# HKUST-Aerial-Robotics/VINS-Mobile

Hardware: AMD Instinct MI355X
Metric: VIO frames/sec (KLT+window solve), 640x480/150 feats/W=10 (higher is better)
Workload: dtype f64 (solve) / u8+i32+f32 (KLT)

## Files before the change

vins-mobile_amd/csrc/vio_frontend.hip:

```cpp
#include <hip/hip_runtime.h>

#include <type_traits>

#include <math.h>
#include <stdint.h>
#include <stdio.h>
#include <string.h>

#include <algorithm>
#include <condition_variable>
#include <memory>
#include <mutex>
#include <thread>
#include <vector>

#include "vio_amd.h"
#include "vio_device.h"
#include "vio_pool.h"

namespace {

constexpr int kMaxLevels = 4;
constexpr int kMaxCap = 512;
constexpr int kWin = 21;
constexpr int kWBits = 14;
constexpr int kMaxRadius = 128;

struct LevelDims {
  int rows[kMaxLevels], cols[kMaxLevels];
  size_t off[kMaxLevels];
  size_t pyr_bytes;
  int levels;
};

__device__ __forceinline__ int reflect101(int p, int len) {
  p = p < 0 ? -p : p;
  p = p >= len ? 2 * len - 2 - p : p;
  return p;
}
__device__ __forceinline__ int descale(int x, int n) { return (x + (1 << (n - 1))) >> n; }

constexpr int kPdW = 64, kPdH = 8;
__global__ __launch_bounds__(256) void pyr_down_kernel(const uint8_t *src_base, uint8_t *dst_base, size_t seq_stride,
                                                       int srows, int scols, int drows, int dcols) {
  constexpr int SW = 2 * kPdW + 4, SH = 2 * kPdH + 4;
  __shared__ int patch[SH][SW + 1];
  __shared__ int hsum[SH][kPdW + 1];
  const uint8_t *src = src_base + (size_t)blockIdx.z * seq_stride;
  uint8_t *dst = dst_base + (size_t)blockIdx.z * seq_stride;
  const int ox = blockIdx.x * kPdW, oy = blockIdx.y * kPdH;
  const int tid = threadIdx.x;
  for (int e = tid; e < SH * SW; e += 256) {
    int ly = e / SW, lx = e - ly * SW;
    int y = reflect101(min(2 * oy + ly - 2, 2 * srows - 2), srows), x = reflect101(min(2 * ox + lx - 2, 2 * scols - 2), scols);
    patch[ly][lx] = src[(size_t)y * scols + x];
  }
  __syncthreads();
  for (int e = tid; e < SH * kPdW; e += 256) {
    int ly = e / kPdW, lx = e - ly * kPdW;
    const int *r = &patch[ly][2 * lx];
    hsum[ly][lx] = r[0] + 4 * r[1] + 6 * r[2] + 4 * r[3] + r[4];
  }
  __syncthreads();
  for (int e = tid; e < kPdH * kPdW; e += 256) {
    int ly = e / kPdW, lx = e - ly * kPdW;
    int x = ox + lx, y = oy + ly;
    if (x < dcols && y < drows) {
      int v = hsum[2 * ly][lx] + 4 * hsum[2 * ly + 1][lx] + 6 * hsum[2 * ly + 2][lx] + 4 * hsum[2 * ly + 3][lx] + hsum[2 * ly + 4][lx];
      dst[(size_t)y * dcols + x] = (uint8_t)((v + 128) >> 8);
    }
  }
}

inline float lk_eps_screen(double eps_sq) { return nextafterf((float)(eps_sq * (1.0 + 1e-5)), INFINITY); }
struct LkParams {
  LevelDims ld;
  int cap;
  int max_count;
  float epsilon_sq_f;
  double epsilon_sq;
  float min_eig;
  const uint8_t *prev0, *next0;
  size_t stride0;
};

__device__ __forceinline__ int wave_sum_i32(int v) {
  v += __builtin_amdgcn_update_dpp(0, v, 0x111, 0xf, 0xf, false);
  v += __builtin_amdgcn_update_dpp(0, v, 0x112, 0xf, 0xf, false);
  v += __builtin_amdgcn_update_dpp(0, v, 0x114, 0xf, 0xf, false);
  v += __builtin_amdgcn_update_dpp(0, v, 0x118, 0xf, 0xf, false);
  v += __builtin_amdgcn_update_dpp(0, v, 0x142, 0xa, 0xf, false);
  v += __builtin_amdgcn_update_dpp(0, v, 0x143, 0xc, 0xf, false);
  return __builtin_amdgcn_readlane(v, 63);
}
__device__ __forceinline__ double wave_sum_exact(int p) {
  int lo = p & 0xffff, hi = p >> 16;
  int slo = wave_sum_i32(lo), shi = wave_sum_i32(hi);
  return (double)shi * 65536.0 + (double)slo;
}

__device__ __forceinline__ void lk_weights(float a, float b, int &iw00, int &iw01, int &iw10, int &iw11) {
  iw00 = __float2int_rn((1.f - a) * (1.f - b) * (1 << kWBits));
  iw01 = __float2int_rn(a * (1.f - b) * (1 << kWBits));
  iw10 = __float2int_rn((1.f - a) * b * (1 << kWBits));
  iw11 = (1 << kWBits) - iw00 - iw01 - iw10;
}

constexpr int kIP = kWin + 3;
constexpr int kDP = kWin + 1;
constexpr int kJMargin = 3;
constexpr int kJP = kWin + 1 + 2 * kJMargin;
constexpr int kJS = 43;
constexpr int kIS = kIP + 1;
struct LkWaveLds {
  union {
    struct {
      uint32_t I[kIP][kIS];
      short2 dI[kDP][kDP];
    };
    uint32_t J[kJP][kJS];
  };
};
typedef short lk_s2 __attribute__((ext_vector_type(2)));
typedef unsigned short lk_us2 __attribute__((ext_vector_type(2)));

struct __attribute__((packed)) LkU32 {
  uint32_t v;
};
__device__ __forceinline__ uint32_t lk_load4(const uint8_t *p) { return reinterpret_cast<const LkU32 *>(p)->v; }
__device__ __forceinline__ void lk_pairs(uint32_t cur, uint32_t next, uint32_t w[4]) {
  w[0] = __builtin_amdgcn_perm(0u, cur, 0x0c010c00u);
  w[1] = __builtin_amdgcn_perm(0u, cur, 0x0c020c01u);
  w[2] = __builtin_amdgcn_perm(0u, cur, 0x0c030c02u);
  w[3] = __builtin_amdgcn_perm(next, cur, 0x0c040c03u);
}

__device__ __forceinline__ void wave_lds_fence() {
  __builtin_amdgcn_fence(__ATOMIC_RELEASE, "wavefront");
  __builtin_amdgcn_wave_barrier();
  __builtin_amdgcn_fence(__ATOMIC_ACQUIRE, "wavefront");
}

__device__ __forceinline__ bool wave_all_small(int p, int q, int r = 0) {
  const bool small = (unsigned)(p + (1 << 24)) < (1u << 25) && (unsigned)(q + (1 << 24)) < (1u << 25) && (unsigned)(r + (1 << 24)) < (1u << 25);
  return __builtin_amdgcn_ballot_w64(!small) == 0ull;
}
__device__ __forceinline__ void wave_sum_exact2(int p, int q, float &sp, float &sq) {
  if (wave_all_small(p, q)) {
    int u[2] = {p, q};
#define VIO_DPPS(ctrl, rmask)                                                  \
  {                                                                            \
    const int t0 = __builtin_amdgcn_update_dpp(0, u[0], ctrl, rmask, 0xf, false); \
    const int t1 = __builtin_amdgcn_update_dpp(0, u[1], ctrl, rmask, 0xf, false); \
    u[0] += t0, u[1] += t1;                                                    \
  }
    VIO_DPPS(0x111, 0xf) VIO_DPPS(0x112, 0xf) VIO_DPPS(0x114, 0xf) VIO_DPPS(0x118, 0xf) VIO_DPPS(0x142, 0xa) VIO_DPPS(0x143, 0xc)
#undef VIO_DPPS
    sp = (float)__builtin_amdgcn_readlane(u[0], 63), sq = (float)__builtin_amdgcn_readlane(u[1], 63);
    return;
  }
  int a = p & 0xffff, b = q & 0xffff, c = p >> 16, d = q >> 16;
#define VIO_DPP4(ctrl, rmask)                                              \
  {                                                                        \
    const int ta = __builtin_amdgcn_update_dpp(0, a, ctrl, rmask, 0xf, false); \
    const int tb = __builtin_amdgcn_update_dpp(0, b, ctrl, rmask, 0xf, false); \
    const int tc = __builtin_amdgcn_update_dpp(0, c, ctrl, rmask, 0xf, false); \
    const int td = __builtin_amdgcn_update_dpp(0, d, ctrl, rmask, 0xf, false); \
    a += ta, b += tb, c += tc, d += td;                                    \
  }
  VIO_DPP4(0x111, 0xf) VIO_DPP4(0x112, 0xf) VIO_DPP4(0x114, 0xf) VIO_DPP4(0x118, 0xf) VIO_DPP4(0x142, 0xa) VIO_DPP4(0x143, 0xc)
#undef VIO_DPP4
  const int sa = __builtin_amdgcn_readlane(a, 63), sb = __builtin_amdgcn_readlane(b, 63), sc = __builtin_amdgcn_readlane(c, 63),
            sd = __builtin_amdgcn_readlane(d, 63);
  sp = (float)sc * 65536.f + (float)sa, sq = (float)sd * 65536.f + (float)sb;
}

__device__ __forceinline__ void wave_sum_exact3(int p, int q, int r, float &sp, float &sq, float &sr) {
  if (wave_all_small(p, q, r)) {
    int w[3] = {p, q, r};
#define VIO_DPPS3(ctrl, rmask)                                                                                       \
  {                                                                                                                   \
    int t[3];                                                                                                         \
    _Pragma("unroll") for (int k = 0; k < 3; k++) t[k] = __builtin_amdgcn_update_dpp(0, w[k], ctrl, rmask, 0xf, false); \
    _Pragma("unroll") for (int k = 0; k < 3; k++) w[k] += t[k];                                                       \
  }
    VIO_DPPS3(0x111, 0xf) VIO_DPPS3(0x112, 0xf) VIO_DPPS3(0x114, 0xf) VIO_DPPS3(0x118, 0xf) VIO_DPPS3(0x142, 0xa) VIO_DPPS3(0x143, 0xc)
#undef VIO_DPPS3
    sp = (float)__builtin_amdgcn_readlane(w[0], 63), sq = (float)__builtin_amdgcn_readlane(w[1], 63), sr = (float)__builtin_amdgcn_readlane(w[2], 63);
    return;
  }
  int u[3] = {p, q, r};
#define VIO_DPPN(N, arr, ctrl, rmask)                                               \
  {                                                                                 \
    int t[N];                                                                       \
    _Pragma("unroll") for (int k = 0; k < N; k++) t[k] = __builtin_amdgcn_update_dpp(0, arr[k], ctrl, rmask, 0xf, false); \
    _Pragma("unroll") for (int k = 0; k < N; k++) arr[k] += t[k];                   \
  }
  VIO_DPPN(3, u, 0x111, 0xf) VIO_DPPN(3, u, 0x112, 0xf) VIO_DPPN(3, u, 0x114, 0xf) VIO_DPPN(3, u, 0x118, 0xf)
  int v[6] = {u[0] & 0xffff, u[1] & 0xffff, u[2] & 0xffff, u[0] >> 16, u[1] >> 16, u[2] >> 16};
  VIO_DPPN(6, v, 0x142, 0xa) VIO_DPPN(6, v, 0x143, 0xc)
#undef VIO_DPPN
  int s[6];
#pragma unroll
  for (int k = 0; k < 6; k++) s[k] = __builtin_amdgcn_readlane(v[k], 63);
  sp = (float)s[3] * 65536.f + (float)s[0], sq = (float)s[4] * 65536.f + (float)s[1], sr = (float)s[5] * 65536.f + (float)s[2];
}

template <bool STATS = false>
__global__ __launch_bounds__(256, 6) void lk_track_kernel(const uint8_t *prev_pyr, const uint8_t *next_pyr, LkParams P,
                                                       const int *n_pts, const float *prev_pts, float *next_pts,
                                                       uint8_t *status, float *err, unsigned long long *stats) {
  __shared__ LkWaveLds lds_all[4];
  const int seq = blockIdx.y;
  const int wave = threadIdx.x >> 6, lane = threadIdx.x & 63;
  const int pt = blockIdx.x * (blockDim.x >> 6) + wave;
  if (pt >= n_pts[seq]) return;
  LkWaveLds &L = lds_all[wave];
  const uint8_t *pp = prev_pyr + (size_t)seq * P.ld.pyr_bytes, *np = next_pyr + (size_t)seq * P.ld.pyr_bytes;
  const size_t pidx = ((size_t)seq * P.cap + pt) * 2;
  const float ptx = prev_pts[pidx], pty = prev_pts[pidx + 1];
  const float half = (kWin - 1) * 0.5f;
  const float FLT_SCALE = 1.f / (1 << 20);
  constexpr int NPX = (kWin * kWin + 63) / 64;
  const int wy0 = min(lane / kWin, 2), wx0 = lane % kWin;
  const int joff = wy0 * kJS + wx0;
  bool st = true;
  float er = 0.f;
  float nxx = 0.f, nxy = 0.f;
  const int max_level = P.ld.levels - 1;
  for (int level = max_level; level >= 0; level--) {
    const int rows = P.ld.rows[level], cols = P.ld.cols[level];
    const uint8_t *I = pp + P.ld.off[level], *J = np + P.ld.off[level];
    if (level == 0) {
      if (P.prev0) I = P.prev0 + (size_t)seq * P.stride0;
      if (P.next0) J = P.next0 + (size_t)seq * P.stride0;
    }
    const float scale = __int_as_float((127 - level) << 23);
    float px = ptx * scale, py = pty * scale;
    float qx, qy;
    if (level == max_level) qx = px, qy = py;
    else qx = nxx * 2.f, qy = nxy * 2.f;
    nxx = qx, nxy = qy;
    px -= half, py -= half;
    int ipx = (int)floorf(px), ipy = (int)floorf(py);
    if (ipx < -kWin || ipx >= cols || ipy < -kWin || ipy >= rows) {
      if (level == 0) st = false, er = 0.f;
      continue;
    }
    float a = px - ipx, b = py - ipy;
    int iw00, iw01, iw10, iw11;
    lk_weights(a, b, iw00, iw01, iw10, iw11);
    wave_lds_fence();
    if (ipx >= 1 && ipx + kIP - 1 <= cols && ipy >= 1 && ipy + kIP - 1 <= rows) {
      const int r = lane / 6, d = lane - 6 * r;
      constexpr int TI = (kIP + 9) / 10;
      uint32_t curs[TI];
#pragma unroll
      for (int t = 0; t < TI; t++) {
        const int ly = r + 10 * t;
        curs[t] = lk_load4(I + (unsigned)(__mul24(ipy - 1 + (ly < kIP ? ly : 0), cols) + ipx - 1 + 4 * d));
      }
#pragma unroll
      for (int t = 0; t < TI; t++) {
        const int ly = r + 10 * t;
        const bool ok = lane < 60 && ly < kIP;
        const uint32_t cur = curs[t];
        uint32_t next = (uint32_t)__builtin_amdgcn_update_dpp(0, (int)cur, 0x130, 0xf, 0xf, false);
        if (d == 5) next = cur >> 24;
        uint32_t w4[4];
        lk_pairs(cur, next, w4);
        if (ok) {
#pragma unroll
          for (int k = 0; k < 4; k++) L.I[ly][4 * d + k] = w4[k];
        }
      }
    } else {
      const int lx = lane & 31;
      const int x = reflect101(ipx - 1 + min(lx, kIP - 1), cols);
      constexpr int RPT = 2, TB = kIP / RPT;
      static_assert(kIP % RPT == 0, "whole trips");
      int vs[TB];
#pragma unroll
      for (int t = 0; t < TB; t++) {
        const int s_y0 = __builtin_amdgcn_readfirstlane(ipy) - 1 + RPT * t;
        const int ro_a = reflect101(s_y0, rows) * cols, ro_b = reflect101(s_y0 + 1, rows) * cols;
        vs[t] = I[(unsigned)(((lane >> 5) ? ro_b : ro_a) + x)];
      }
#pragma unroll
      for (int t = 0; t < TB; t++) {
        const int ly = (lane >> 5) + RPT * t, v = vs[t];
        const int vr = __builtin_amdgcn_update_dpp(0, v, 0x130, 0xf, 0xf, false);
        if (lx < kIP) L.I[ly][lx] = (uint32_t)v | ((uint32_t)vr << 16);
      }
    }
    wave_lds_fence();
    constexpr int SEG = 5, NSEG = 5, NCP = kDP / 2;
    static_assert(kDP % 2 == 0 && NCP * NSEG <= 64 && SEG * NSEG >= kDP && kDP >= SEG, "column pairs x segments");
    const bool inside = ipx >= 0 && ipx + kDP <= cols && ipy >= 0 && ipy + kDP <= rows;
    if (lane < NCP * NSEG) {
      const int seg = lane / NCP, cp = lane - NCP * seg, c = 2 * cp;
      const int r0 = seg * SEG < kDP - SEG ? seg * SEG : kDP - SEG;
      const uint32_t *Ip = &L.I[0][0] + (__mul24(r0, kIS) + c);
      uint32_t *Dp = reinterpret_cast<uint32_t *>(&L.dI[0][0]) + (__mul24(r0, kDP) + c);
      const lk_s2 k3 = {3, 3}, k10 = {10, 10};
      auto walk = [&](auto checked) {
        const unsigned ok0 = (unsigned)(ipx + c) < (unsigned)cols, ok1 = (unsigned)(ipx + c + 1) < (unsigned)cols;
        lk_s2 P0[SEG + 2], P1[SEG + 2], P2[SEG + 2];
#pragma unroll
        for (int r = 0; r < SEG + 2; r++)
          __builtin_memcpy(&P0[r], Ip + r * kIS, 4), __builtin_memcpy(&P1[r], Ip + r * kIS + 1, 4), __builtin_memcpy(&P2[r], Ip + r * kIS + 2, 4);
        lk_s2 h[SEG + 2], v[SEG + 2];
#pragma unroll
        for (int r = 0; r < SEG + 2; r++) h[r] = P2[r] - P0[r], v[r] = (P0[r] + P2[r]) * k3 + P1[r] * k10;
#pragma unroll
        for (int r = 2; r < SEG + 2; r++) {
          const lk_s2 dx = (h[r - 2] + h[r]) * k3 + h[r - 1] * k10, dy = v[r] - v[r - 2];
          uint32_t ux, uy;
          __builtin_memcpy(&ux, &dx, 4), __builtin_memcpy(&uy, &dy, 4);
          uint32_t d0 = __builtin_amdgcn_perm(uy, ux, 0x05040100u), d1 = __builtin_amdgcn_perm(uy, ux, 0x07060302u);
          if (decltype(checked)::value) {
            const unsigned rok = (unsigned)(ipy + r0 + r - 2) < (unsigned)rows;
            d0 &= 0u - (ok0 & rok), d1 &= 0u - (ok1 & rok);
          }
          Dp[(r - 2) * kDP] = d0, Dp[(r - 2) * kDP + 1] = d1;
        }
      };
      if (inside) walk(std::false_type{});
      else walk(std::true_type{});
    }
    wave_lds_fence();
    constexpr int NPP = (NPX + 1) / 2;
    const lk_s2 sw_top = {(short)iw00, (short)iw01}, sw_bot = {(short)iw10, (short)iw11};
    lk_s2 IxP[NPP], IyP[NPP];
    int Ic[NPX];
    int p11 = 0, p12 = 0, p22 = 0;
#pragma unroll
    for (int h = 0; h < NPP; h++) IxP[h] = IyP[h] = lk_s2{0, 0};
#pragma unroll
    for (int q = 0; q < NPX; q++) {
      const int y = wy0 + 3 * q, x = wx0;
      lk_s2 it, ib;
      __builtin_memcpy(&it, &L.I[y + 1][x + 1], 4);
      __builtin_memcpy(&ib, &L.I[y + 2][x + 1], 4);
      const int ival = __builtin_amdgcn_sdot2(it, sw_top, __builtin_amdgcn_sdot2(ib, sw_bot, 1 << (kWBits - 5 - 1), false), false) >> (kWBits - 5);
      uint32_t d00, d01, d10, d11;
      __builtin_memcpy(&d00, &L.dI[y][x], 4), __builtin_memcpy(&d01, &L.dI[y][x + 1], 4);
      __builtin_memcpy(&d10, &L.dI[y + 1][x], 4), __builtin_memcpy(&d11, &L.dI[y + 1][x + 1], 4);
      const uint32_t xt = __builtin_amdgcn_perm(d01, d00, 0x05040100u), yt = __builtin_amdgcn_perm(d01, d00, 0x07060302u);
      const uint32_t xb = __builtin_amdgcn_perm(d11, d10, 0x05040100u), yb = __builtin_amdgcn_perm(d11, d10, 0x07060302u);
      lk_s2 sxt, syt, sxb, syb;
      __builtin_memcpy(&sxt, &xt, 4), __builtin_memcpy(&syt, &yt, 4), __builtin_memcpy(&sxb, &xb, 4), __builtin_memcpy(&syb, &yb, 4);
      int ixval = __builtin_amdgcn_sdot2(sxt, sw_top, __builtin_amdgcn_sdot2(sxb, sw_bot, 1 << (kWBits - 1), false), false) >> kWBits;
      int iyval = __builtin_amdgcn_sdot2(syt, sw_top, __builtin_amdgcn_sdot2(syb, sw_bot, 1 << (kWBits - 1), false), false) >> kWBits;
      if (lane >= 3 * kWin) ixval = iyval = 0;
      Ic[q] = (1 << (kWBits - 5 - 1)) - (int)((unsigned)ival << (kWBits - 5));
      if (q & 1) IxP[q >> 1].y = (short)ixval, IyP[q >> 1].y = (short)iyval;
      else IxP[q >> 1].x = (short)ixval, IyP[q >> 1].x = (short)iyval;
      p11 += ixval * ixval, p12 += ixval * iyval, p22 += iyval * iyval;
    }
    float f11, f12, f22;
    wave_sum_exact3(p11, p12, p22, f11, f12, f22);
    float A11 = f11 * FLT_SCALE, A12 = f12 * FLT_SCALE, A22 = f22 * FLT_SCALE;
    float D = A11 * A22 - A12 * A12;
    float minEig = (A22 + A11 - sqrtf((A11 - A22) * (A11 - A22) + 4.f * A12 * A12)) / (2 * kWin * kWin);
    if (minEig < P.min_eig || D < 1.1920929e-07f) {
      if (level == 0) st = false;
      continue;
    }
    D = 1.f / D;
    qx -= half, qy -= half;
    float pdx = 0.f, pdy = 0.f;
    int jox = 0, joy = 0;
    bool j_staged = false;
    auto stage_j = [&](int iqx, int iqy) {
      jox = iqx - kJMargin, joy = iqy - kJMargin;
      wave_lds_fence();
      if (jox >= 0 && jox + kJP <= cols && joy >= 0 && joy + kJP <= rows) {
        const int r = lane / 7, d = lane - 7 * r;
        constexpr int TJ = (kJP + 8) / 9;
        uint32_t curs[TJ];
#pragma unroll
        for (int t = 0; t < TJ; t++) {
          const int ly = r + 9 * t;
          curs[t] = lk_load4(J + (unsigned)(__mul24(joy + (ly < kJP ? ly : 0), cols) + jox + 4 * d));
        }
#pragma unroll
        for (int t = 0; t < TJ; t++) {
          const int ly = r + 9 * t;
          const bool ok = lane < 63 && ly < kJP;
          const uint32_t cur = curs[t];
          uint32_t next = (uint32_t)__builtin_amdgcn_update_dpp(0, (int)cur, 0x130, 0xf, 0xf, false);
          if (d == 6) next = cur >> 24;
          uint32_t w4[4];
          lk_pairs(cur, next, w4);
          if (ok) {
#pragma unroll
            for (int k = 0; k < 4; k++) L.J[ly][4 * d + k] = w4[k];
          }
        }
      } else {
        const int lx = lane & 31;
        const int x = reflect101(min(max(jox + min(lx, kJP - 1), -cols + 1), 2 * cols - 2), cols);
        constexpr int RPT = 2, TB = kJP / RPT;
        static_assert(kJP % RPT == 0, "whole trips");
        int vs[TB];
#pragma unroll
        for (int t = 0; t < TB; t++) {
          const int s_y0 = __builtin_amdgcn_readfirstlane(joy) + RPT * t;
          const int ro_a = reflect101(min(max(s_y0, -rows + 1), 2 * rows - 2), rows) * cols;
          const int ro_b = reflect101(min(max(s_y0 + 1, -rows + 1), 2 * rows - 2), rows) * cols;
          vs[t] = J[(unsigned)(((lane >> 5) ? ro_b : ro_a) + x)];
        }
#pragma unroll
        for (int t = 0; t < TB; t++) {
          const int ly = (lane >> 5) + RPT * t, v = vs[t];
          const int vr = __builtin_amdgcn_update_dpp(0, v, 0x130, 0xf, 0xf, false);
          if (lx < kJP) L.J[ly][lx] = (uint32_t)v | ((uint32_t)vr << 16);
        }
      }
      wave_lds_fence();
      j_staged = true;
    };
    const uint32_t *Jl = &L.J[0][0];
    auto diff_j = [&](int base, int q, lk_us2 wtop, lk_s2 wbot) {
      lk_us2 top;
      lk_s2 bot;
      const int o = base + (joff + 3 * q * kJS);
      const uint32_t t32 = Jl[o], b32 = Jl[o + kJS];
      __builtin_memcpy(&top, &t32, 4);
      __builtin_memcpy(&bot, &b32, 4);
      return __builtin_amdgcn_sdot2(bot, wbot, (int)__builtin_amdgcn_udot2(top, wtop, (unsigned)Ic[q], false), false) >> (kWBits - 5);
    };
    int nit = 0;
    for (int j = 0; j < P.max_count; j++) {
      int iqx = (int)floorf(qx), iqy = (int)floorf(qy);
      if (iqx < -kWin || iqx >= cols || iqy < -kWin || iqy >= rows) {
        if (level == 0) st = false;
        break;
      }
      if (STATS) nit++;
      if (!j_staged || iqx < jox || iqx > jox + 2 * kJMargin || iqy < joy || iqy > joy + 2 * kJMargin) stage_j(iqx, iqy);
      a = qx - iqx, b = qy - iqy;
      lk_weights(a, b, iw00, iw01, iw10, iw11);
      int pb1 = 0, pb2 = 0;
      const lk_us2 wtop = {(unsigned short)iw00, (unsigned short)iw01};
      const lk_s2 wbot = {(short)iw10, (short)iw11};
      const int jbase = __mul24(iqy - joy, kJS) + (iqx - jox);
#pragma unroll
      for (int h = 0; h < NPP; h++) {
        const int d0 = diff_j(jbase, 2 * h, wtop, wbot), d1 = 2 * h + 1 < NPX ? diff_j(jbase, 2 * h + 1, wtop, wbot) : 0;
        const unsigned pk = __builtin_amdgcn_perm((unsigned)d1, (unsigned)d0, 0x05040100u);
        lk_s2 dp;
        __builtin_memcpy(&dp, &pk, 4);
        pb1 = __builtin_amdgcn_sdot2(dp, IxP[h], pb1, false), pb2 = __builtin_amdgcn_sdot2(dp, IyP[h], pb2, false);
      }
      float fb1, fb2;
      wave_sum_exact2(pb1, pb2, fb1, fb2);
      float b1 = fb1 * FLT_SCALE, b2 = fb2 * FLT_SCALE;
      float ddx = (A12 * b2 - A22 * b1) * D, ddy = (A12 * b1 - A11 * b2) * D;
      qx += ddx, qy += ddy;
      nxx = qx + half, nxy = qy + half;
      if (!(ddx * ddx + ddy * ddy > P.epsilon_sq_f) && (double)ddx * ddx + (double)ddy * ddy <= P.epsilon_sq) break;
      constexpr float kCentiUp = 0.010000000707805157f;
      static_assert((double)kCentiUp > 0.01 && (double)0.01f < 0.01, "float neighbours of 0.01");
      if (j > 0 && fabsf(ddx + pdx) < kCentiUp && fabsf(ddy + pdy) < kCentiUp) {
        nxx -= ddx * 0.5f, nxy -= ddy * 0.5f;
        break;
      }
      pdx = ddx, pdy = ddy;
    }
    if (STATS && lane == 0) {
      unsigned long long *sl = stats + ((blockIdx.x + 7 * blockIdx.y) & 63) * 16;
      atomicAdd(sl + level, (unsigned long long)nit);
      atomicAdd(sl + P.ld.levels + level, 1ull);
    }
    if (st && level == 0) {
      float ex = nxx - half, ey = nxy - half;
      int iex = (int)floorf(ex), iey = (int)floorf(ey);
      if (iex < -kWin || iex >= cols || iey < -kWin || iey >= rows) {
        st = false;
        continue;
      }
      if (!j_staged || iex < jox || iex > jox + 2 * kJMargin || iey < joy || iey > joy + 2 * kJMargin) stage_j(iex, iey);
      float aa = ex - iex, bb = ey - iey;
      lk_weights(aa, bb, iw00, iw01, iw10, iw11);
      int pe = 0;
      const lk_us2 wtop = {(unsigned short)iw00, (unsigned short)iw01};
      const lk_s2 wbot = {(short)iw10, (short)iw11};
      const int jbase = __mul24(iey - joy, kJS) + (iex - jox);
#pragma unroll
      for (int q = 0; q < NPX; q++) {
        const int d = abs(diff_j(jbase, q, wtop, wbot));
        pe += lane < 3 * kWin ? d : 0;
      }
      const int se = wave_sum_i32(pe);
      er = (float)se * 1.f / (32 * kWin * kWin);
    }
  }
  if (lane == 0) {
    next_pts[pidx] = nxx, next_pts[pidx + 1] = nxy;
    status[(size_t)seq * P.cap + pt] = st ? 1 : 0;
    err[(size_t)seq * P.cap + pt] = er;
  }
}

__device__ int solve_cubic_dev(const double c[4], double r[3]) {
  double a0 = c[0], a1 = c[1], a2 = c[2], a3 = c[3];
  double x0 = 0, x1 = 0, x2 = 0;
  int n = 0;
  if (a0 == 0) {
    if (a1 == 0) {
      if (a2 == 0) n = a3 == 0 ? -1 : 0;
      else x0 = -a3 / a2, n = 1;
    } else {
      double d = a2 * a2 - 4 * a1 * a3;
      if (d >= 0) {
        d = sqrt(d);
        double q1 = (-a2 + d) * 0.5, q2 = (a2 + d) * -0.5;
        if (fabs(q1) > fabs(q2)) x0 = q1 / a1, x1 = a3 / q1;
        else x0 = q2 / a1, x1 = a3 / q2;
        n = d > 0 ? 2 : 1;
      }
    }
  } else {
    a0 = 1. / a0, a1 *= a0, a2 *= a0, a3 *= a0;
    double Q = (a1 * a1 - 3 * a2) * (1. / 9), R = (2 * a1 * a1 * a1 - 9 * a1 * a2 + 27 * a3) * (1. / 54);
    double Qcubed = Q * Q * Q, d = Qcubed - R * R;
    const double kPi = 3.14159265358979323846;
    if (d >= 0) {
      double theta = acos(R / sqrt(Qcubed)), sqrtQ = sqrt(Q);
      double t0 = -2 * sqrtQ, t1 = theta * (1. / 3), t2 = a1 * (1. / 3);
      x0 = t0 * cos(t1) - t2, x1 = t0 * cos(t1 + (2. * kPi / 3)) - t2, x2 = t0 * cos(t1 + (4. * kPi / 3)) - t2;
      n = 3;
    } else {
      d = sqrt(-d);
      double e = pow(d + fabs(R), 0.333333333333);
      if (R > 0) e = -e;
      x0 = (e + Q / e) - a1 * (1. / 3);
      n = 1;
    }
  }
  r[0] = x0, r[1] = x1, r[2] = x2;
  return n;
}

struct SevenPointWork {
  double a[63], f1[9], f2[9];
  int colperm[10];
};

__device__ __forceinline__ int run7point_group(const float *ms1, const float *ms2, double *fmatrix, SevenPointWork &wk, int l) {
  double *a = wk.a, *f1 = wk.f1, *f2 = wk.f2;
  int *colperm = wk.colperm;
  auto group_sync = [] {
    __builtin_amdgcn_fence(__ATOMIC_RELEASE, "wavefront");
    __builtin_amdgcn_wave_barrier();
    __builtin_amdgcn_fence(__ATOMIC_ACQUIRE, "wavefront");
  };
  if (l < 7) {
    double x0 = ms1[2 * l], y0 = ms1[2 * l + 1], x1 = ms2[2 * l], y1 = ms2[2 * l + 1];
    double *row = a + l * 9;
    row[0] = x1 * x0, row[1] = x1 * y0, row[2] = x1, row[3] = y1 * x0, row[4] = y1 * y0, row[5] = y1, row[6] = x0,
    row[7] = y0, row[8] = 1;
  }
  if (l < 9) colperm[l] = l;
  group_sync();
  for (int k = 0; k < 7; k++) {
    double best = -1;
    int bpos = k * 9 + k;
#pragma unroll
    for (int q = 0; q < 4; q++) {
      const int e = l + 16 * q, i = e / 9, j = e - 9 * i;
      if (e < 63 && i >= k && j >= k) {
        const double v = fabs(a[e]);
        if (v > best) best = v, bpos = e;
      }
    }
#pragma unroll
    for (int m = 1; m < 16; m <<= 1) {
      const double ob = __shfl_xor(best, m, 16);
      const int op = __shfl_xor(bpos, m, 16);
      if (ob > best || (ob == best && op < bpos)) best = ob, bpos = op;
    }
    const int pr = bpos / 9, pc = bpos - 9 * pr;
    if (pr != k && l < 9) {
      const double t = a[k * 9 + l];
      a[k * 9 + l] = a[pr * 9 + l], a[pr * 9 + l] = t;
    }
    group_sync();
    if (pc != k) {
      if (l < 7) {
        const double t = a[l * 9 + k];
        a[l * 9 + k] = a[l * 9 + pc], a[l * 9 + pc] = t;
      }
      if (l == 15) {
        const int t = colperm[k];
        colperm[k] = colperm[pc], colperm[pc] = t;
      }
    }
    group_sync();
    const double d = a[k * 9 + k];
    group_sync();
    if (d == 0.0) continue;
    if (l < 9) a[k * 9 + l] /= d;
    group_sync();
    double fv[4], pv[4], av[4];
    int ev[4];
#pragma unroll
    for (int q = 0; q < 4; q++) {
      const int e = l + 16 * q, ii = e / 9, j = e - 9 * ii, i = ii < k ? ii : ii + 1;
      const bool on = e < 54;
      ev[q] = on ? i * 9 + j : -1;
      fv[q] = on ? a[i * 9 + k] : 0.0, pv[q] = on ? a[k * 9 + j] : 0.0, av[q] = on ? a[i * 9 + j] : 0.0;
    }
    group_sync();
#pragma unroll
    for (int q = 0; q < 4; q++)
      if (ev[q] >= 0 && fv[q] != 0.0) a[ev[q]] = av[q] - fv[q] * pv[q];
    group_sync();
  }
  if (l < 9) {
#pragma unroll
    for (int q = 0; q < 2; q++) {
      double *out = q == 0 ? f1 : f2;
      const double vj = l < 7 ? -a[l * 9 + 7 + q] : (l - 7 == q ? 1.0 : 0.0);
      out[colperm[l]] = vj;
    }
  }
  group_sync();
  if (l < 9) f1[l] -= f2[l];
  group_sync();
  int n = 0;
  if (l == 0) {
    double c[4], r[3];
    double t0 = f2[4] * f2[8] - f2[5] * f2[7], t1 = f2[3] * f2[8] - f2[5] * f2[6], t2 = f2[3] * f2[7] - f2[4] * f2[6];
    c[3] = f2[0] * t0 - f2[1] * t1 + f2[2] * t2;
    c[2] = f1[0] * t0 - f1[1] * t1 + f1[2] * t2 - f1[3] * (f2[1] * f2[8] - f2[2] * f2[7]) +
           f1[4] * (f2[0] * f2[8] - f2[2] * f2[6]) - f1[5] * (f2[0] * f2[7] - f2[1] * f2[6]) +
           f1[6] * (f2[1] * f2[5] - f2[2] * f2[4]) - f1[7] * (f2[0] * f2[5] - f2[2] * f2[3]) +
           f1[8] * (f2[0] * f2[4] - f2[1] * f2[3]);
    t0 = f1[4] * f1[8] - f1[5] * f1[7], t1 = f1[3] * f1[8] - f1[5] * f1[6], t2 = f1[3] * f1[7] - f1[4] * f1[6];
    c[1] = f2[0] * t0 - f2[1] * t1 + f2[2] * t2 - f2[3] * (f1[1] * f1[8] - f1[2] * f1[7]) +
           f2[4] * (f1[0] * f1[8] - f1[2] * f1[6]) - f2[5] * (f1[0] * f1[7] - f1[1] * f1[6]) +
           f2[6] * (f1[1] * f1[5] - f1[2] * f1[4]) - f2[7] * (f1[0] * f1[5] - f1[2] * f1[3]) +
           f2[8] * (f1[0] * f1[4] - f1[1] * f1[3]);
    c[0] = f1[0] * t0 - f1[1] * t1 + f1[2] * t2;
    n = solve_cubic_dev(c, r);
    if (n >= 1 && n <= 3)
      for (int k = 0; k < n; k++, fmatrix += 9) {
        double lambda = r[k], mu = 1., s = f1[8] * r[k] + f2[8];
        if (fabs(s) > 2.220446049250313e-16) mu = 1. / s, lambda *= mu, fmatrix[8] = 1.;
        else fmatrix[8] = 0.;
        for (int i = 0; i < 8; i++) fmatrix[i] = f1[i] * lambda + f2[i] * mu;
      }
  }
  return __shfl(n, 0, 16);
}

__device__ __forceinline__ float epipolar_error(const double *F, float x1f, float y1f, float x2f, float y2f) {
  double x1 = x1f, y1 = y1f, x2 = x2f, y2 = y2f;
  double a = F[0] * x1 + F[1] * y1 + F[2], b = F[3] * x1 + F[4] * y1 + F[5], c = F[6] * x1 + F[7] * y1 + F[8];
  double s2 = 1. / (a * a + b * b);
  double d2 = x2 * a + y2 * b + c;
  a = F[0] * x2 + F[3] * y2 + F[6], b = F[1] * x2 + F[4] * y2 + F[7], c = F[2] * x2 + F[5] * y2 + F[8];
  double s1 = 1. / (a * a + b * b);
  double d1 = x1 * a + y1 * b + c;
  return (float)fmax(d1 * d1 * s1, d2 * d2 * s2);
}
__device__ __forceinline__ bool epipolar_inlier(const double *F, float x1f, float y1f, float x2f, float y2f, float t) {
  return epipolar_error(F, x1f, y1f, x2f, y2f) <= t;
}

__device__ bool have_collinear_dev(const float *p, int count) {
  int i = count - 1;
  for (int j = 0; j < i; j++) {
    double dx1 = p[2 * j] - p[2 * i], dy1 = p[2 * j + 1] - p[2 * i + 1];
    for (int k = 0; k < j; k++) {
      double dx2 = p[2 * k] - p[2 * i], dy2 = p[2 * k + 1] - p[2 * i + 1];
      if (fabs(dx2 * dy1 - dy2 * dx1) <= 1.1920929e-07 * (fabs(dx1) + fabs(dy1) + fabs(dx2) + fabs(dy2))) return true;
    }
  }
  return false;
}

__device__ int ransac_update_iters(double p, double ep, int model_points, int max_iters) {
  p = fmax(p, 0.), p = fmin(p, 1.), ep = fmax(ep, 0.), ep = fmin(ep, 1.);
  double num = fmax(1. - p, 2.2250738585072014e-308), denom = 1. - pow(1. - ep, (double)model_points);
  if (denom < 2.2250738585072014e-308) return 0;
  num = log(num), denom = log(denom);
  return denom >= 0 || -num >= max_iters * (-denom) ? max_iters : (int)rint(num / denom);
}

constexpr int kHypBatch = 16;

struct RansacShared {
  SevenPointWork work[kHypBatch];
  float ms1[kHypBatch][14], ms2[kHypBatch][14];
  double F[kHypBatch][27];
  int nmodels[kHypBatch];
  int good[kHypBatch][3];
  int idx[kHypBatch][7];
  int valid[kHypBatch];
  int coll[kHypBatch];
  unsigned long long rng_before[kHypBatch];
  unsigned long long rng_state;
  int niters, max_good, best_h, best_k, iter, done, failed_first;
  double bestF[9];
  double med[kHypBatch][3], min_median;
};

template <class MaskT>
__device__ void fundamental_ransac_block(RansacShared &S, const float *m1, const float *m2, int count, float thresh,
                                         double confidence, MaskT *mask, long long *prof = nullptr) {
  const int tid = threadIdx.x, nt = blockDim.x;
  long long pt = prof ? clock64() : 0;
#define RS_STAMP(k)                                                    \
  do {                                                                 \
    if (prof && tid == 0) {                                            \
      const long long now = clock64();                                 \
      prof[k] += now - pt, pt = now;                                   \
    }                                                                  \
  } while (0)
  const int model_points = 7, max_iters = 1000;
  const bool lmeds = count < 15;
  if (count < 8) {
    for (int i = tid; i < count; i += nt) mask[i] = 1;
    __syncthreads();
    return;
  }
  if (tid == 0) {
    S.rng_state = 0xffffffffffffffffULL;
    S.niters = lmeds ? ransac_update_iters(confidence, 0.45, model_points, max_iters) : max_iters;
    S.max_good = 0, S.best_h = -1, S.best_k = 0, S.iter = 0, S.done = 0, S.failed_first = 0;
    S.min_median = 1.7976931348623157e308;
  }
  __syncthreads();
  const float t = thresh * thresh;
  while (true) {
    const int nb = (!lmeds && S.iter == 0) ? 8 : kHypBatch;
    auto draw = [&](unsigned long long &st, int h, bool with_check) {
      int idx[7], i = 0, iters = 0;
      const int max_attempts = 10000;
      for (; iters < max_attempts; iters++) {
        for (i = 0; i < model_points && iters < max_attempts;) {
          int idx_i = 0;
          for (;;) {
            st = (unsigned long long)(unsigned)st * 4164903690U + (unsigned)(st >> 32);
            idx_i = idx[i] = (int)((unsigned)st % (unsigned)count);
            int j;
            for (j = 0; j < i; j++)
              if (idx_i == idx[j]) break;
            if (j == i) break;
          }
          S.ms1[h][2 * i] = m1[2 * idx_i], S.ms1[h][2 * i + 1] = m1[2 * idx_i + 1];
          S.ms2[h][2 * i] = m2[2 * idx_i], S.ms2[h][2 * i + 1] = m2[2 * idx_i + 1];
          i++;
        }
        if (with_check && i == model_points && (have_collinear_dev(S.ms1[h], i) || have_collinear_dev(S.ms2[h], i))) continue;
        break;
      }
      return (i == model_points && iters < max_attempts) ? 1 : 0;
    };
    if (tid == 0) {
      const unsigned ucount = (unsigned)count, magic = 0xffffffffu / ucount;
      unsigned long long st = S.rng_state;
      for (int h = 0; h < nb; h++) {
        S.rng_before[h] = st;
        int idx[7];
#pragma unroll
        for (int i = 0; i < 7; i++) {
          for (;;) {
            st = (unsigned long long)(unsigned)st * 4164903690U + (unsigned)(st >> 32);
            const unsigned x = (unsigned)st;
            unsigned r = x - __umulhi(x, magic) * ucount;
            r = r >= ucount ? r - ucount : r;
            r = r >= ucount ? r - ucount : r;
            bool dup = false;
#pragma unroll
            for (int j = 0; j < i; j++) dup |= (int)r == idx[j];
            if (!dup) { idx[i] = (int)r; break; }
          }
          S.idx[h][i] = idx[i];
        }
        S.valid[h] = 1;
      }
      S.rng_state = st;
    }
    __syncthreads();
    RS_STAMP(0);
    for (int it = tid; it < nb * 7; it += nt) {
      const int h = it / 7, i = it - 7 * h, id = S.idx[h][i];
      S.ms1[h][2 * i] = m1[2 * id], S.ms1[h][2 * i + 1] = m1[2 * id + 1];
      S.ms2[h][2 * i] = m2[2 * id], S.ms2[h][2 * i + 1] = m2[2 * id + 1];
    }
    __syncthreads();
    if (tid < nb) S.coll[tid] = (have_collinear_dev(S.ms1[tid], 7) || have_collinear_dev(S.ms2[tid], 7)) ? 1 : 0;
    __syncthreads();
    if (tid == 0) {
      int first = -1;
      for (int h = 0; h < nb && first < 0; h++)
        if (S.coll[h]) first = h;
      if (first >= 0) {
        unsigned long long st = S.rng_before[first];
        for (int h = first; h < nb; h++) {
          S.valid[h] = draw(st, h, true);
          if (!S.valid[h]) {
            for (int hh = h + 1; hh < nb; hh++) S.valid[hh] = 0;
            break;
          }
        }
        S.rng_state = st;
      }
    }
    __syncthreads();
    RS_STAMP(1);
    for (int h = tid >> 4; h < nb; h += nt >> 4) {
      int n = 0;
      if (S.valid[h]) n = run7point_group(S.ms1[h], S.ms2[h], S.F[h], S.work[h], tid & 15);
      if ((tid & 15) == 0) {
        S.nmodels[h] = n < 0 ? 0 : n;
        S.good[h][0] = S.good[h][1] = S.good[h][2] = 0;
      }
    }
    __syncthreads();
    RS_STAMP(2);
    if (lmeds) {
      for (int hk = tid; hk < nb * 3; hk += nt) {
        const int h = hk / 3, k = hk - 3 * h;
        if (k >= S.nmodels[h]) continue;
        int bits[14];
        for (int i = 0; i < count; i++) {
          const int b = __float_as_int(epipolar_error(S.F[h] + 9 * k, m1[2 * i], m1[2 * i + 1], m2[2 * i], m2[2 * i + 1]));
          int j = i;
          for (; j > 0 && bits[j - 1] > b; j--) bits[j] = bits[j - 1];
          bits[j] = b;
        }
        S.med[h][k] = (count & 1) ? (double)__int_as_float(bits[count / 2])
                                  : (double)(__int_as_float(bits[count / 2 - 1]) + __int_as_float(bits[count / 2])) * 0.5;
      }
    } else
    for (int item = tid; item < nb * 3 * count; item += nt) {
      int hk = item / count, i = item - hk * count;
      int h = hk / 3, k = hk - 3 * h;
      if (k < S.nmodels[h] && epipolar_inlier(S.F[h] + 9 * k, m1[2 * i], m1[2 * i + 1], m2[2 * i], m2[2 * i + 1], t))
        atomicAdd(&S.good[h][k], 1);
    }
    __syncthreads();
    RS_STAMP(3);
    if (tid == 0) {
      for (int h = 0; h < nb; h++) {
        if (S.iter >= S.niters) { S.done = 1; break; }
        if (!S.valid[h]) {
          if (S.iter == 0) S.failed_first = 1;
          S.done = 1;
          break;
        }
        for (int k = 0; k < S.nmodels[h]; k++) {
          if (lmeds) {
            if (S.med[h][k] < S.min_median) {
              S.min_median = S.med[h][k];
              for (int q = 0; q < 9; q++) S.bestF[q] = S.F[h][9 * k + q];
            }
            continue;
          }
          int good = S.good[h][k];
          if (good > max(S.max_good, model_points - 1)) {
            S.max_good = good;
            for (int q = 0; q < 9; q++) S.bestF[q] = S.F[h][9 * k + q];
            S.best_h = h;
            S.niters = ransac_update_iters(confidence, (double)(count - good) / count, model_points, S.niters);
          }
        }
        S.iter++;
      }
      if (S.iter >= S.niters) S.done = 1;
    }
    __syncthreads();
    RS_STAMP(4);
    if (prof && tid == 0) prof[6] += 1;
    if (S.done) break;
  }
  if (lmeds && S.min_median < 1.7976931348623157e308 && !S.failed_first) {
    double sigma = 2.5 * 1.4826 * (1 + 5. / (count - model_points)) * sqrt(S.min_median);
    sigma = fmax(sigma, 0.001);
    const float ts = (float)(sigma * sigma);
    for (int i = tid; i < count; i += nt)
      mask[i] = epipolar_inlier(S.bestF, m1[2 * i], m1[2 * i + 1], m2[2 * i], m2[2 * i + 1], ts) ? 1 : 0;
  } else if (!lmeds && S.max_good > 0 && !S.failed_first) {
    for (int i = tid; i < count; i += nt)
      mask[i] = epipolar_inlier(S.bestF, m1[2 * i], m1[2 * i + 1], m2[2 * i], m2[2 * i + 1], t) ? 1 : 0;
  } else {
    for (int i = tid; i < count; i += nt) mask[i] = 1;
  }
  __syncthreads();
  RS_STAMP(5);
#undef RS_STAMP
}

struct TrackerArrays {
  int cap;
  int rows, cols;
  float *cur_pts, *pre_pts, *forw_pts;
  int *ids, *track_cnt;
  int *n_pts;
  int *n_forw;
  int *n_id;
  uint8_t *lk_status;
  int *kept_xy;
  int *n_kept;
  float *pnp_pts;
  int *pnp_ids, *n_pnp;
  const int *hw;
  int radius;
  float f_thresh;
  double f_conf;
  long long *prof;
};

template <int CAP>
struct TrackShared {
  float pre[CAP][2], cur[CAP][2], forw[CAP][2];
  int ids[CAP], cnt[CAP];
  int keep[CAP];
  int pos[CAP];
  float t_pre[CAP][2], t_cur[CAP][2], t_forw[CAP][2];
  int t_ids[CAP], t_cnt[CAP];
  int n;
  int order[CAP];
  int ixy[CAP][2];
  unsigned long long inside[CAP][CAP / 64];
  int hw[2 * kMaxRadius + 1];
};

template <int CAP>
__device__ void compact_block(TrackShared<CAP> &T) {
  const int tid = threadIdx.x, nt = blockDim.x;
  const int n = T.n;
  __syncthreads();
  {
    __shared__ int s_wcnt[16];
    const int wave = tid >> 6, lane = tid & 63, nwv = nt >> 6;
    int running = 0;
    for (int base = 0; base < n; base += nt) {
      const int i = base + tid;
      const bool k = i < n && T.keep[i];
      const unsigned long long b = __builtin_amdgcn_ballot_w64(k);
      if (lane == 0) s_wcnt[wave] = __builtin_popcountll(b);
      __syncthreads();
      int off = running, total = 0;
      for (int w = 0; w < nwv; w++) {
        const int c = s_wcnt[w];
        if (w < wave) off += c;
        total += c;
      }
      if (i < n) T.pos[i] = off + __builtin_popcountll(b & ((1ull << lane) - 1ull));
      running += total;
      __syncthreads();
    }
    if (tid == 0) T.n = running;
  }
  __syncthreads();
  for (int i = tid; i < n; i += nt)
    if (T.keep[i]) {
      int p = T.pos[i];
      T.t_pre[p][0] = T.pre[i][0], T.t_pre[p][1] = T.pre[i][1];
      T.t_cur[p][0] = T.cur[i][0], T.t_cur[p][1] = T.cur[i][1];
      T.t_forw[p][0] = T.forw[i][0], T.t_forw[p][1] = T.forw[i][1];
      T.t_ids[p] = T.ids[i], T.t_cnt[p] = T.cnt[i];
    }
  __syncthreads();
  for (int i = tid; i < T.n; i += nt) {
    T.pre[i][0] = T.t_pre[i][0], T.pre[i][1] = T.t_pre[i][1];
    T.cur[i][0] = T.t_cur[i][0], T.cur[i][1] = T.t_cur[i][1];
    T.forw[i][0] = T.t_forw[i][0], T.forw[i][1] = T.t_forw[i][1];
    T.ids[i] = T.t_ids[i], T.cnt[i] = T.t_cnt[i];
  }
  __syncthreads();
}

template <int CAP>
__global__ __launch_bounds__(256, 2) void track_update_kernel(TrackerArrays A, int publish) {
  extern __shared__ __attribute__((aligned(16))) unsigned char smem_raw[];
  TrackShared<CAP> &T = *reinterpret_cast<TrackShared<CAP> *>(smem_raw);
  RansacShared &R = *reinterpret_cast<RansacShared *>(smem_raw + ((sizeof(TrackShared<CAP>) + 15) & ~(size_t)15));
  const int seq = blockIdx.x, tid = threadIdx.x, nt = blockDim.x;
  const size_t base = (size_t)seq * A.cap;
  const int n0 = A.n_pts[seq];
#define TU_STAMP(k)                                                  \
  do {                                                               \
    if (A.prof && seq == 0 && tid == 0) A.prof[k] = clock64();       \
  } while (0)
  TU_STAMP(0);
  if (tid == 0) T.n = n0;
  for (int i = tid; i < n0; i += nt) {
    T.pre[i][0] = A.pre_pts[(base + i) * 2], T.pre[i][1] = A.pre_pts[(base + i) * 2 + 1];
    T.cur[i][0] = A.cur_pts[(base + i) * 2], T.cur[i][1] = A.cur_pts[(base + i) * 2 + 1];
    T.forw[i][0] = A.forw_pts[(base + i) * 2], T.forw[i][1] = A.forw_pts[(base + i) * 2 + 1];
    T.ids[i] = A.ids[base + i], T.cnt[i] = A.track_cnt[base + i];
    int ix = __float2int_rn(T.forw[i][0]), iy = __float2int_rn(T.forw[i][1]);
    bool inb = 1 <= ix && ix < A.cols - 1 && 1 <= iy && iy < A.rows - 1;
    T.keep[i] = (A.lk_status[base + i] && inb) ? 1 : 0;
  }
  __syncthreads();
  TU_STAMP(1);
  if (n0 > 0) {
    compact_block(T);
    TU_STAMP(2);
    if (T.n >= 8) {
      fundamental_ransac_block(R, &T.cur[0][0], &T.forw[0][0], T.n, A.f_thresh, A.f_conf, T.keep, A.prof && seq == 0 ? A.prof + 16 : nullptr);
      TU_STAMP(3);
      compact_block(T);
    }
  }
  TU_STAMP(4);
  for (int i = tid; i < T.n; i += nt) {
    A.pnp_pts[(base + i) * 2] = T.forw[i][0], A.pnp_pts[(base + i) * 2 + 1] = T.forw[i][1];
    A.pnp_ids[base + i] = T.ids[i];
  }
  if (tid == 0) A.n_pnp[seq] = T.n;
  if (publish) {
    if (T.n >= 8) {
      TU_STAMP(5);
      fundamental_ransac_block(R, &T.pre[0][0], &T.forw[0][0], T.n, A.f_thresh, A.f_conf, T.keep, A.prof && seq == 0 ? A.prof + 24 : nullptr);
      TU_STAMP(6);
      compact_block(T);
    }
    TU_STAMP(7);
    const int n = T.n;
    for (int i = tid; i < n; i += nt) {
      T.cnt[i] += 1;
      T.ixy[i][0] = __float2int_rn(T.forw[i][0]), T.ixy[i][1] = __float2int_rn(T.forw[i][1]);
    }
    __syncthreads();
    for (int i = tid; i < n; i += nt) {
      int rank = 0, ci = T.cnt[i];
      for (int j = 0; j < n; j++) rank += (T.cnt[j] > ci || (T.cnt[j] == ci && j < i)) ? 1 : 0;
      T.order[rank] = i;
    }
    const int words = (n + 63) / 64;
    __syncthreads();
    TU_STAMP(8);
    for (int q = tid; q < 2 * A.radius + 1; q += nt) T.hw[q] = A.hw[q];
    __syncthreads();
    {
      const int wave = tid >> 6, lane = tid & 63, nwv = nt >> 6;
      constexpr int kW = CAP / 64;
      int jx[kW], jy[kW];
#pragma unroll
      for (int w = 0; w < kW; w++) {
        const int j = min(64 * w + lane, n - 1);
        jx[w] = T.ixy[j][0], jy[w] = T.ixy[j][1];
      }
      const int rad = A.radius;
      for (int i = wave; i < n; i += nwv) {
        const int ix = T.ixy[i][0], iy = T.ixy[i][1];
#pragma unroll
        for (int w = 0; w < kW; w++) {
          if (w < words) {
            const int dy = iy - jy[w], dx = ix - jx[w];
            const int h = T.hw[rad + min(max(dy, -rad), rad)];
            const bool in = 64 * w + lane < n && dy >= -rad && dy <= rad && dx >= -h && dx <= h;
            const unsigned long long bits = __builtin_amdgcn_ballot_w64(in);
            if (lane == 0) T.inside[i][w] = bits;
          }
        }
      }
    }
    __syncthreads();
    TU_STAMP(9);
    if (tid < 64) {
      const int lane = tid;
      unsigned long long mine = 0;
      int c = 0;
      for (int r0 = 0; r0 < n; r0 += 64) {
        const int my_i = r0 + lane < n ? T.order[r0 + lane] : 0;
        const int cnt = n - r0 < 64 ? n - r0 : 64;
        unsigned long long kept = 0;
        for (int q0 = 0; q0 < cnt; q0 += 8) {
          int is[8];
          unsigned long long rows[8];
#pragma unroll
          for (int u = 0; u < 8; u++) {
            is[u] = __builtin_amdgcn_readlane(my_i, (q0 + u) & 63);
            rows[u] = lane < words ? T.inside[is[u]][lane] : 0ull;
          }
#pragma unroll
          for (int u = 0; u < 8; u++) {
            const int i = is[u];
            const bool keep_it = q0 + u < cnt && __builtin_amdgcn_ballot_w64((rows[u] & mine) != 0) == 0;
            const unsigned long long bit = keep_it ? 1ULL << (i & 63) : 0ull;
            mine |= lane == (i >> 6) ? bit : 0ull;
            kept |= (unsigned long long)keep_it << ((q0 + u) & 63);
          }
        }
        if (lane < cnt) {
          const bool k = (kept >> lane) & 1ull;
          T.keep[my_i] = k ? 1 : 0;
          if (k) T.pos[my_i] = c + __builtin_popcountll(kept & ((1ull << lane) - 1ull));
        }
        c += __builtin_popcountll(kept);
      }
      if (lane == 0) T.n = c;
    }
    __syncthreads();
    TU_STAMP(10);
    for (int i = tid; i < n; i += nt)
      if (T.keep[i]) {
        int p = T.pos[i];
        T.t_forw[p][0] = T.forw[i][0], T.t_forw[p][1] = T.forw[i][1];
        T.t_ids[p] = T.ids[i], T.t_cnt[p] = T.cnt[i];
        A.kept_xy[(base + p) * 2] = T.ixy[i][0], A.kept_xy[(base + p) * 2 + 1] = T.ixy[i][1];
      }
    __syncthreads();
    for (int i = tid; i < T.n; i += nt) {
      T.forw[i][0] = T.t_forw[i][0], T.forw[i][1] = T.t_forw[i][1];
      T.ids[i] = T.t_ids[i], T.cnt[i] = T.t_cnt[i];
    }
    if (tid == 0) A.n_kept[seq] = T.n;
    __syncthreads();
  }
  const int n = T.n;
  for (int i = tid; i < n; i += nt) {
    A.forw_pts[(base + i) * 2] = T.forw[i][0], A.forw_pts[(base + i) * 2 + 1] = T.forw[i][1];
    A.ids[base + i] = T.ids[i], A.track_cnt[base + i] = T.cnt[i];
    if (!publish) {
      A.pre_pts[(base + i) * 2] = T.pre[i][0], A.pre_pts[(base + i) * 2 + 1] = T.pre[i][1];
      A.cur_pts[(base + i) * 2] = T.forw[i][0], A.cur_pts[(base + i) * 2 + 1] = T.forw[i][1];
    }
  }
  if (tid == 0) {
    A.n_forw[seq] = n;
    if (!publish) A.n_pts[seq] = n;
  }
  TU_STAMP(11);
#undef TU_STAMP
}

__device__ __forceinline__ unsigned ordered_bits(float v) {
  unsigned u = __float_as_uint(v);
  return (u & 0x80000000u) ? ~u : (u | 0x80000000u);
}
__device__ __forceinline__ float from_ordered_bits(unsigned u) {
  return __uint_as_float((u & 0x80000000u) ? (u & 0x7fffffffu) : ~u);
}

constexpr int kDetW = 60;
constexpr int kDetWaves = 4;
constexpr int kDetR = 32;

template <int CTRL>
__device__ __forceinline__ float dpp_f32(float v) {
  return __int_as_float(__builtin_amdgcn_update_dpp(0, __float_as_int(v), CTRL, 0xf, 0xf, true));
}
#define LANE_LEFT(v) dpp_f32<0x138>(v)
#define LANE_RIGHT(v) dpp_f32<0x130>(v)

__device__ __forceinline__ float sqrt_rn_normal(float x) {
  const float r = __builtin_amdgcn_sqrtf(x);
  const float rm = __int_as_float(__float_as_int(r) - 1), rp = __int_as_float(__float_as_int(r) + 1);
  const float em = __builtin_fmaf(-rm, r, x), ep = __builtin_fmaf(-rp, r, x);
  float y = em <= 0.f ? rm : r;
  y = ep > 0.f ? rp : y;
  return y;
}

template <bool IMG_MASK>
__global__ __launch_bounds__(256) void detect_kernel(const uint8_t *img_base, size_t img_stride, const uint8_t *mask_base,
                                                     size_t mask_stride, const int *kept_xy, const int *n_kept, int cap,
                                                     const int *hw, int radius, unsigned *max_bits, int rows, int cols,
                                                     unsigned long long *cand_base, int seg_cap, int *n_cand, const int *n_have,
                                                     int max_corners) {
  if (n_have && n_have[blockIdx.z] >= max_corners) return;
  constexpr int kCandLds = kDetWaves * kDetW * kDetR / 4 + 64;
  __shared__ unsigned long long s_mask[kDetWaves][kDetR];
  __shared__ unsigned long long s_cand[kCandLds];
  __shared__ unsigned smax;
  __shared__ int s_ncand, s_base, s_ndisc;
  __shared__ int2 s_disc[kMaxCap];
  const int seq = blockIdx.z, tid = threadIdx.x, wave = tid >> 6, lane = tid & 63;
  const uint8_t *img = img_base + (size_t)seq * img_stride;
  const int XB = blockIdx.x * (kDetWaves * kDetW), Y0 = blockIdx.y * kDetR;
  const int X0 = XB + wave * kDetW;
  if (tid == 0) smax = 0, s_ncand = 0, s_ndisc = 0;
  if (tid < kDetWaves * kDetR) s_mask[tid / kDetR][tid % kDetR] = 0ull;
  __syncthreads();
  if (!IMG_MASK) {
    const int nk = n_kept[seq];
    for (int k = tid; k < nk; k += 256) {
      const int cx = kept_xy[((size_t)seq * cap + k) * 2], cy = kept_xy[((size_t)seq * cap + k) * 2 + 1];
      if (cy + radius >= Y0 && cy - radius < Y0 + kDetR && cx + radius >= XB - 2 && cx - radius < XB + kDetWaves * kDetW + 2) {
        const int slot = atomicAdd(&s_ndisc, 1);
        s_disc[slot] = make_int2(cx, cy);
      }
    }
    __syncthreads();
    const int nd = s_ndisc;
    for (int it = tid; it < nd * kDetR * kDetWaves; it += 256) {
      const int wv = it % kDetWaves, r = (it / kDetWaves) % kDetR, dsc = it / (kDetWaves * kDetR);
      const int cx = s_disc[dsc].x, dy = Y0 + r - s_disc[dsc].y;
      if (dy < -radius || dy > radius) continue;
      const int h = hw[radius + dy];
      const int l0 = max(cx - h - (XB + wv * kDetW - 2), 0), l1 = min(cx + h - (XB + wv * kDetW - 2), 63);
      if (l0 > l1) continue;
      const unsigned long long bits = (l1 - l0 == 63 ? ~0ull : ((1ull << (l1 - l0 + 1)) - 1ull)) << l0;
      atomicOr(&s_mask[wv][r], bits);
    }
    __syncthreads();
  }
  const float s = (float)(1.0 / (4.0 * 3.0 * 255.0));
  const float s2 = s * 2.f;
  const __amdgpu_buffer_rsrc_t img_rsrc = __builtin_amdgcn_make_buffer_rsrc((void *)img, 0, rows * cols, 0x00020000);
  const int xe = X0 - 2 + lane;
  const int xr = reflect101(min(max(xe, -cols + 1), 2 * cols - 2), cols);
  const int xm = reflect101(xr - 1, cols), xp = reflect101(xr + 1, cols);
  float D[3] = {0.f, 0.f, 0.f}, T[3] = {0.f, 0.f, 0.f};
  float Hxx[3] = {0.f, 0.f, 0.f}, Hxy[3] = {0.f, 0.f, 0.f}, Hyy[3] = {0.f, 0.f, 0.f};
  float E[3] = {0.f, 0.f, 0.f};
  float my_max = -INFINITY;
  int prev_yr = -1, prev_yp = -1;
  const bool out_lane = lane >= 2 && lane < 2 + kDetW && xe < cols;
  static_assert((kDetR + 4) % 3 == 0, "the row loop is unrolled by the rotation period");
  unsigned RB[3][3] = {{0u, 0u, 0u}, {0u, 0u, 0u}, {0u, 0u, 0u}};
  const bool inner_rows = Y0 - 3 >= 0 && Y0 + kDetR + 2 <= rows - 1;
  auto strip = [&](auto inner_tag) {
  constexpr bool INNER = decltype(inner_tag)::value;
  auto entering_row = [&](int step) {
    if (INNER) return Y0 - 1 + step;
    const int yr_ = reflect101(min(max(Y0 - 2 + step, -rows + 1), 2 * rows - 2), rows);
    return reflect101(yr_ + 1, rows);
  };
  auto fetch_raw = [&](int y, unsigned (&b)[3]) {
    const int ro = __builtin_amdgcn_readfirstlane(y * cols);
    b[0] = __builtin_amdgcn_raw_buffer_load_b8(img_rsrc, xm, ro, 0), b[1] = __builtin_amdgcn_raw_buffer_load_b8(img_rsrc, xr, ro, 0),
    b[2] = __builtin_amdgcn_raw_buffer_load_b8(img_rsrc, xp, ro, 0);
  };
  fetch_raw(entering_row(0), RB[2]);
  auto three_steps = [&](int s0, auto head_tag) {
    constexpr bool HEAD = decltype(head_tag)::value;
#pragma unroll
    for (int u = 0; u < 3; u++) {
      const int step = s0 + u;
      const int jn = u, jm = (u + 1) % 3, jr = (u + 2) % 3;
      const int ye = Y0 - 2 + step;
      const int yr = INNER ? ye : reflect101(min(max(ye, -rows + 1), 2 * rows - 2), rows);
      const int ym = INNER ? ye - 1 : reflect101(yr - 1, rows), yp = INNER ? ye + 1 : reflect101(yr + 1, rows);
      auto row_dt = [&](int y, float &d, float &t) {
        const int ro = __builtin_amdgcn_readfirstlane(y * cols);
        const float a0 = (float)__builtin_amdgcn_raw_buffer_load_b8(img_rsrc, xm, ro, 0), a1 = (float)__builtin_amdgcn_raw_buffer_load_b8(img_rsrc, xr, ro, 0),
                    a2 = (float)__builtin_amdgcn_raw_buffer_load_b8(img_rsrc, xp, ro, 0);
        d = a2 - a0;
        t = s2 * a1 + s * (a0 + a2);
      };
      if (INNER ? step == 0 : !(step > 0 && ym == prev_yr && yr == prev_yp)) row_dt(ym, D[jm], T[jm]), row_dt(yr, D[jr], T[jr]);
      if (step + 1 < kDetR + 4) fetch_raw(entering_row(step + 1), RB[jn]);
      {
        const float a0 = (float)RB[jr][0], a1 = (float)RB[jr][1], a2 = (float)RB[jr][2];
        D[jn] = a2 - a0;
        T[jn] = s2 * a1 + s * (a0 + a2);
      }
      prev_yr = yr, prev_yp = yp;
      const float dx = s2 * D[jr] + s * (D[jm] + D[jn]);
      const float dy = T[jn] - T[jm];
      const float pxx = dx * dx, pxy = dx * dy, pyy = dy * dy;
      Hxx[jn] = (LANE_LEFT(pxx) + pxx) + LANE_RIGHT(pxx);
      Hxy[jn] = (LANE_LEFT(pxy) + pxy) + LANE_RIGHT(pxy);
      Hyy[jn] = (LANE_LEFT(pyy) + pyy) + LANE_RIGHT(pyy);
      float e2 = 0.f;
      if (!HEAD || step >= 2) {
        const float a = ((Hxx[jm] + Hxx[jr]) + Hxx[jn]) * 0.5f;
        const float b = (Hxy[jm] + Hxy[jr]) + Hxy[jn];
        const float c = ((Hyy[jm] + Hyy[jr]) + Hyy[jn]) * 0.5f;
        e2 = (a + c) - sqrt_rn_normal((a - c) * (a - c) + b * b);
      }
      E[jn] = e2;
      if (!HEAD || step >= 4) {
        const int y = ye - 2, r = step - 4;
        float m = fmaxf(fmaxf(E[jm], E[jr]), E[jn]);
        m = fmaxf(m, fmaxf(LANE_LEFT(m), LANE_RIGHT(m)));
        if (out_lane && (INNER || y < rows)) {
          const float v = E[jr];
          bool unmasked;
          if (IMG_MASK) unmasked = mask_base[(size_t)seq * mask_stride + (size_t)y * cols + xe] != 0;
          else unmasked = ((s_mask[wave][r] >> lane) & 1ull) == 0ull;
          if (unmasked) {
            my_max = fmaxf(my_max, v);
            if (xe >= 1 && xe < cols - 1 && (INNER || (y >= 1 && y < rows - 1)) && v > 0.f && v == m) {
              const int slot = atomicAdd(&s_ncand, 1);
              const unsigned idx = (unsigned)y << 16 | (unsigned)xe;
              if (slot < kCandLds) s_cand[slot] = ((unsigned long long)__float_as_uint(v) << 32) | (0xffffffffu - idx);
            }
          }
        }
      }
    }
  };
  static_assert(kDetR + 4 > 6 && (kDetR + 4) % 6 == 0, "two head rounds, then rounds of six steps");
  three_steps(0, std::true_type{}), three_steps(3, std::true_type{});
#pragma unroll 1
  for (int s0 = 6; s0 < kDetR + 4; s0 += 6) three_steps(s0, std::false_type{}), three_steps(s0 + 3, std::false_type{});
  };
  if (inner_rows) strip(std::true_type{});
  else strip(std::false_type{});
  {
    unsigned m = my_max == -INFINITY ? 0u : ordered_bits(my_max);
#pragma unroll
    for (int o = 32; o > 0; o >>= 1) m = max(m, (unsigned)__shfl_xor((int)m, o, 64));
    if (lane == 0 && m) atomicMax(&smax, m);
  }
  __syncthreads();
  const int nseg = gridDim.y;
  const size_t segi = (size_t)seq * nseg + blockIdx.y;
  const int nc = min(s_ncand, kCandLds);
  if (tid == 0 && nc) s_base = atomicAdd(&n_cand[segi], nc);
  __syncthreads();
  for (int i = tid; i < nc; i += 256) {
    const int slot = s_base + i;
    if (slot < seg_cap) cand_base[segi * seg_cap + slot] = s_cand[i];
  }
  if (tid == 0 && smax) atomicMax(&max_bits[segi], smax);
}

#undef LANE_LEFT
#undef LANE_RIGHT

struct SelectParams {
  int cap, rows, cols, max_corners;
  float min_dist;
  double fx, fy, cx, cy;
};

constexpr int kSelThreads = 512;
constexpr int kSelMaxSeg = 256;
constexpr int kSelLds = 8192;

__device__ __forceinline__ unsigned long long wave_max_u64(unsigned long long v) {
#pragma unroll
  for (int o = 32; o > 0; o >>= 1) {
    unsigned long long t = __shfl_xor(v, o, 64);
    v = t > v ? t : v;
  }
  return v;
}

__global__ __launch_bounds__(kSelThreads) void corner_select_kernel(unsigned long long *cand_base, int seg_cap, int nseg,
                                                                    int *n_cand, unsigned *max_bits,
                                                                    double quality, SelectParams P, float *forw_pts,
                                                                    float *cur_pts, float *pre_pts, int *ids, int *track_cnt,
                                                                    int *n_forw, int *n_pts, int *n_id, VioObs *obs,
                                                                    int *n_obs) {
  __shared__ unsigned long long keys[kSelLds];
  __shared__ unsigned long long red[kSelThreads / 64];
  __shared__ int s_n, s_cnt;
  __shared__ int s_off[kSelMaxSeg + 1];
  const int seq = blockIdx.x, tid = threadIdx.x, nt = blockDim.x;
  unsigned long long *cand = cand_base + (size_t)seq * nseg * seg_cap;
  const size_t base = (size_t)seq * P.cap;
  int n = n_forw[seq];
  const int want = P.max_corners - n;
  const float md2 = P.min_dist * P.min_dist;
  unsigned mb = 0;
  for (int g = 0; g < nseg; g++) mb = max(mb, max_bits[(size_t)seq * nseg + g]);
  const float thr = mb ? (float)((double)from_ordered_bits(mb) * quality) : 3.4e38f;
  if (tid == 0) s_n = n, s_cnt = 0;
  __syncthreads();
  if (tid == 0) {
    int o = 0;
    for (int g = 0; g < nseg; g++) s_off[g] = o, o += min(n_cand[(size_t)seq * nseg + g], seg_cap);
    s_off[nseg] = o;
  }
  __syncthreads();
  const int real = s_off[nseg];
  for (int i = tid; i < real; i += nt) {
    int g = 0;
    while (s_off[g + 1] <= i) g++;
    const unsigned long long k = cand[(size_t)g * seg_cap + (i - s_off[g])];
    if (k && __uint_as_float((unsigned)(k >> 32)) > thr) {
      int slot = atomicAdd(&s_cnt, 1);
      if (slot < kSelLds) keys[slot] = k;
    }
  }
  __syncthreads();
  for (int g = tid; g < nseg; g += nt) n_cand[(size_t)seq * nseg + g] = 0, max_bits[(size_t)seq * nseg + g] = 0;
  if (s_cnt > kSelLds) {
    __shared__ unsigned long long smax[kSelMaxSeg];
    __shared__ unsigned long long part[kSelThreads / 64][4];
    const int wv = tid >> 6, nwv = nt >> 6;
    auto rescan = [&](int g0, int ng, int bx, int by, bool first) {
      unsigned long long m[4] = {0, 0, 0, 0};
#pragma unroll
      for (int q = 0; q < 4; q++) {
        if (q >= ng) continue;
        unsigned long long *seg = cand + (size_t)(g0 + q) * seg_cap;
        const int cnt = s_off[g0 + q + 1] - s_off[g0 + q];
        for (int j = tid; j < cnt; j += nt) {
          const unsigned long long c = seg[j];
          if (!c) continue;
          bool dead;
          if (first) {
            dead = !(__uint_as_float((unsigned)(c >> 32)) > thr);
          } else if (P.min_dist >= 1.f) {
            const unsigned idx = 0xffffffffu - (unsigned)(c & 0xffffffffu);
            const float dx = (float)((int)(idx & 0xffffu) - bx), dy = (float)((int)(idx >> 16) - by);
            dead = dx * dx + dy * dy < md2;
          } else {
            const unsigned idx = 0xffffffffu - (unsigned)(c & 0xffffffffu);
            dead = (int)(idx & 0xffffu) == bx && (int)(idx >> 16) == by;
          }
          if (dead) seg[j] = 0;
          else m[q] = c > m[q] ? c : m[q];
        }
      }
#pragma unroll
      for (int q = 0; q < 4; q++) {
        const unsigned long long x = wave_max_u64(m[q]);
        if ((tid & 63) == 0) part[wv][q] = x;
      }
      __syncthreads();
      if (tid < ng) {
        unsigned long long x = part[0][tid];
        for (int w2 = 1; w2 < nwv; w2++) x = part[w2][tid] > x ? part[w2][tid] : x;
        smax[g0 + tid] = x;
      }
      __syncthreads();
    };
    for (int g0 = 0; g0 < nseg; g0 += 4) rescan(g0, min(4, nseg - g0), 0, 0, true);
    const int reach = P.min_dist >= 1.f ? (int)ceilf(P.min_dist) : 0;
    for (int round = 0; round < want; round++) {
      unsigned long long best = 0;
      for (int g = tid & 63; g < nseg; g += 64) best = smax[g] > best ? smax[g] : best;
      best = wave_max_u64(best);
      if (best == 0) break;
      const unsigned bidx = 0xffffffffu - (unsigned)(best & 0xffffffffu);
      const int bx = bidx & 0xffffu, by = bidx >> 16;
      if (tid == 0) {
        int p = s_n++;
        forw_pts[(base + p) * 2] = (float)bx, forw_pts[(base + p) * 2 + 1] = (float)by;
        ids[base + p] = -1, track_cnt[base + p] = 1;
      }
      const int glo = max(0, (by - reach) / kDetR), ghi = min(nseg - 1, (by + reach) / kDetR);
      for (int g0 = glo; g0 <= ghi; g0 += 4) rescan(g0, min(4, ghi - g0 + 1), bx, by, false);
    }
  } else {
  unsigned long long *K = keys;
  const int nc = s_cnt;
  unsigned long long mine = 0;
  for (int i = tid; i < nc; i += nt) {
    const unsigned long long k = K[i];
    mine = k > mine ? k : mine;
  }
  for (int round = 0; round < want; round++) {
    unsigned long long best = wave_max_u64(mine);
    if ((tid & 63) == 0) red[tid >> 6] = best;
    __syncthreads();
    best = red[0];
    for (int w = 1; w < nt / 64; w++) best = red[w] > best ? red[w] : best;
    __syncthreads();
    if (best == 0) break;
    const unsigned bidx = 0xffffffffu - (unsigned)(best & 0xffffffffu);
    const int bx = bidx & 0xffffu, by = bidx >> 16;
    if (tid == 0) {
      int p = s_n++;
      forw_pts[(base + p) * 2] = (float)bx, forw_pts[(base + p) * 2 + 1] = (float)by;
      ids[base + p] = -1, track_cnt[base + p] = 1;
    }
    mine = 0;
    if (P.min_dist >= 1.f) {
      for (int i = tid; i < nc; i += nt) {
        const unsigned long long c = K[i];
        if (c) {
          const unsigned idx = 0xffffffffu - (unsigned)(c & 0xffffffffu);
          const float dx = (float)((int)(idx & 0xffffu) - bx), dy = (float)((int)(idx >> 16) - by);
          if (dx * dx + dy * dy < md2) K[i] = 0;
          else mine = c > mine ? c : mine;
        }
      }
    } else {
      for (int i = tid; i < nc; i += nt) {
        const unsigned long long c = K[i];
        if (c == best) K[i] = 0;
        else mine = c > mine ? c : mine;
      }
    }
  }
  }
  __syncthreads();
  n = s_n;
  if (tid == 0) {
    int nid = n_id[seq];
    for (int i = 0; i < n; i++)
      if (ids[base + i] == -1) ids[base + i] = nid++;
    n_id[seq] = nid;
    n_forw[seq] = n, n_pts[seq] = n, n_obs[seq] = n;
  }
  __syncthreads();
  for (int i = tid; i < n; i += nt) {
    float x = forw_pts[(base + i) * 2], y = forw_pts[(base + i) * 2 + 1];
    cur_pts[(base + i) * 2] = x, cur_pts[(base + i) * 2 + 1] = y;
    pre_pts[(base + i) * 2] = x, pre_pts[(base + i) * 2 + 1] = y;
    VioObs o;
    o.id = ids[base + i];
    o.x = ((double)x - P.cx) / P.fx, o.y = ((double)y - P.cy) / P.fy, o.z = 1.0;
    obs[base + i] = o;
  }
}

void circle_halfwidths(int radius, std::vector<int> &hw) {
  hw.assign(2 * radius + 1, -1);
  int err = 0, dx = radius, dy = 0, plus = 1, minus = (radius << 1) - 1;
  while (dx >= dy) {
    hw[radius + dy] = std::max(hw[radius + dy], dx), hw[radius - dy] = std::max(hw[radius - dy], dx);
    hw[radius + dx] = std::max(hw[radius + dx], dy), hw[radius - dx] = std::max(hw[radius - dx], dy);
    dy++;
    err += plus;
    plus += 2;
    int mask = (err <= 0) - 1;
    err -= minus & mask;
    dx += mask;
    minus -= mask & 2;
  }
}

}

using vio::DevBuf;
using vio::PinnedBuf;

struct vio_frontend {
  int device = -1;
  VioConfig cfg;
  int n_seq = 0, cap = 0;
  LevelDims ld;
  hipStream_t stream = nullptr;
  DevBuf<uint8_t> pyr[2];
  int cur_idx = 0;
  bool have_img = false;
  const uint8_t *lvl0[2] = {nullptr, nullptr};
  DevBuf<uint8_t> mask;
  DevBuf<unsigned> max_bits;
  DevBuf<unsigned long long> cand;
  int nseg = 0, seg_cap = 0;
  DevBuf<int> n_cand;
  DevBuf<float> cur_pts, pre_pts, forw_pts, lk_err;
  DevBuf<unsigned long long> lk_stats;
  bool lk_stats_on = false;
  DevBuf<int> ids, track_cnt, n_pts, n_forw, n_id, kept_xy, n_kept, hw, n_obs, pnp_ids, n_pnp;
  DevBuf<float> pnp_pts;
  DevBuf<uint8_t> lk_status;
  DevBuf<VioObs> obs;
  DevBuf<long long> d_prof;
  bool attr_set = false;
  bool detect_always = false;
  DevBuf<uint8_t> frames;
  int n_frames = 0;
  vio::LaunchTimer timer;
  DevBuf<uint8_t> d_stage;
  PinnedBuf<VioObs> p_obs;
  PinnedBuf<int> p_nobs;
  PinnedBuf<uint8_t> p_frames;
  bool pending = false, pending_publish = false;
  bool pending_async = false;
  struct Async {
    std::thread th;
    std::mutex m;
    std::condition_variable cv;
    bool has_job = false, busy = false, quit = false;
    const uint8_t *gray = nullptr;
    int rows = 0, cols = 0, stride = 0, publish = 0, rc = VIO_OK;
  } *async = nullptr;
  std::vector<VioObs> h_obs;
  std::vector<int> h_nobs;
  ~vio_frontend() {
    if (async) {
      {
        std::lock_guard<std::mutex> lk(async->m);
        async->quit = true;
      }
      async->cv.notify_all();
      if (async->th.joinable()) async->th.join();
      delete async;
    }
    (void)hipDeviceSynchronize();
    if (stream) (void)hipStreamDestroy(stream);
  }
};

namespace {

constexpr int kPd4H = 16, kPd4Dw = (2 * kPdW + 8) / 4;
constexpr int kPd4T = 3;
template <bool COPY>
__global__ __launch_bounds__(256) void pyr_down4_kernel(const uint8_t *src_base, size_t src_stride, uint8_t *dst_base, size_t seq_stride,
                                                        int srows, int scols, int drows, int dcols, uint8_t *copy_base) {
  constexpr int SH = 2 * kPd4H + 4;
  constexpr int NE = (SH * kPd4Dw + 255) / 256;
  __shared__ uint32_t raw[SH][kPd4Dw + 1];
  __shared__ uint32_t hsum[SH / 2][kPdW + 1];
  const uint8_t *src = src_base + (size_t)blockIdx.z * src_stride;
  uint8_t *dst = dst_base + (size_t)blockIdx.z * seq_stride;
  const int ox = blockIdx.x * kPdW;
  const int tid = threadIdx.x;
  const int ndw = scols >> 2, dw0 = (2 * ox - 4) >> 2;
  int e_ly[NE], e_d[NE];
  bool e_ok[NE];
#pragma unroll
  for (int i = 0; i < NE; i++) {
    const int e = tid + 256 * i;
    e_ok[i] = e < SH * kPd4Dw;
    const int ec = e_ok[i] ? e : 0;
    e_ly[i] = ec / kPd4Dw;
    e_d[i] = min(max(dw0 + ec - e_ly[i] * kPd4Dw, 0), ndw - 1);
  }
  const int tile0 = blockIdx.y * kPd4T;
  auto fetch = [&](int oy, uint32_t (&v)[NE]) {
#pragma unroll
    for (int i = 0; i < NE; i++) {
      const int y = reflect101(min(2 * oy + e_ly[i] - 2, 2 * srows - 2), srows);
      v[i] = reinterpret_cast<const uint32_t *>(src + (size_t)y * scols)[e_d[i]];
    }
  };
  uint32_t cur[NE], nxt[NE];
  fetch(tile0 * kPd4H, cur);
#pragma unroll 1
  for (int t = 0; t < kPd4T; t++) {
    const int oy = (tile0 + t) * kPd4H;
    if (oy >= drows) break;
    const bool more = t + 1 < kPd4T && oy + kPd4H < drows;
    if (more) fetch(oy + kPd4H, nxt);
#pragma unroll
    for (int i = 0; i < NE; i++) {
      if (!e_ok[i]) continue;
      const int ly = e_ly[i], lx = tid + 256 * i - ly * kPd4Dw;
      raw[ly][lx] = cur[i];
      if (COPY) {
        const int yy = 2 * oy + ly - 2, dd = dw0 + lx;
        if (ly >= 2 && ly < SH - 2 && lx >= 1 && lx <= (2 * kPdW) / 4 && yy < srows && dd < ndw)
          reinterpret_cast<uint32_t *>(copy_base + (size_t)blockIdx.z * seq_stride + (size_t)yy * scols)[dd] = cur[i];
      }
    }
    __syncthreads();
    if (tid < SH) {
      if (ox == 0) {
        const uint32_t d1 = raw[tid][1];
        raw[tid][0] = ((d1 >> 16) & 0xffu) << 16 | ((d1 >> 8) & 0xffu) << 24;
      }
      const int lr = ndw - dw0;
      if (lr >= 1 && lr < kPd4Dw) {
        const uint32_t dl = raw[tid][lr - 1];
        raw[tid][lr] = ((dl >> 16) & 0xffu) | ((dl >> 8) & 0xffu) << 8;
      }
    }
    __syncthreads();
    for (int e = tid; e < (SH / 2) * kPdW; e += 256) {
      const int p = e / kPdW, lx = e - p * kPdW;
      const int b = 2 * lx + 2, dwi = b >> 2, sh = (b & 3) * 8;
      auto hrow = [&](int ly) {
        const uint32_t lo = raw[ly][dwi], hi = raw[ly][dwi + 1];
        return __builtin_amdgcn_udot4(__builtin_amdgcn_alignbit(hi, lo, sh), 0x04060401u, __builtin_amdgcn_ubfe(hi, sh, 8), false);
      };
      hsum[p][lx] = hrow(2 * p) | hrow(2 * p + 1) << 16;
    }
    __syncthreads();
    {
      const int ly = tid >> 4, lx = (tid & 15) * 4;
      const int x = ox + lx, y = oy + ly;
      if (x < dcols && y < drows) {
        uint32_t out = 0;
        const lk_us2 w14 = {1, 4}, w64 = {6, 4};
#pragma unroll
        for (int i = 0; i < 4; i++) {
          lk_us2 p0, p1;
          __builtin_memcpy(&p0, &hsum[ly][lx + i], 4), __builtin_memcpy(&p1, &hsum[ly + 1][lx + i], 4);
          const uint32_t v = __builtin_amdgcn_udot2(p0, w14, __builtin_amdgcn_udot2(p1, w64, hsum[ly + 2][lx + i] & 0xffffu, false), false);
          out |= ((v + 128) >> 8) << (8 * i);
        }
        *reinterpret_cast<uint32_t *>(dst + (size_t)y * dcols + x) = out;
      }
    }
    if (!more) break;
#pragma unroll
    for (int i = 0; i < NE; i++) cur[i] = nxt[i];
  }
}

__global__ __launch_bounds__(256) void copy_frames_kernel(const uint8_t *src, size_t src_stride, uint8_t *dst,
                                                          size_t dst_stride, size_t bytes, int vec_ok) {
  const int seq = blockIdx.y;
  const uint8_t *sp = src + (size_t)seq * src_stride;
  uint8_t *dp = dst + (size_t)seq * dst_stride;
  const size_t i = (size_t)blockIdx.x * blockDim.x + threadIdx.x;
  if (vec_ok) {
    if (i * 16 < bytes) reinterpret_cast<uint4 *>(dp)[i] = reinterpret_cast<const uint4 *>(sp)[i];
  } else {
    const size_t b0 = i * 16, b1 = b0 + 16 < bytes ? b0 + 16 : bytes;
    for (size_t b = b0; b < b1; b++) dp[b] = sp[b];
  }
}

int launch_track_update(vio_frontend *fe, int publish, hipStream_t st) {
  TrackerArrays A;
  A.cap = fe->cap, A.rows = fe->cfg.image_rows, A.cols = fe->cfg.image_cols;
  A.cur_pts = fe->cur_pts.p, A.pre_pts = fe->pre_pts.p, A.forw_pts = fe->forw_pts.p, A.ids = fe->ids.p, A.track_cnt = fe->track_cnt.p;
  A.n_pts = fe->n_pts.p, A.n_forw = fe->n_forw.p, A.n_id = fe->n_id.p, A.lk_status = fe->lk_status.p, A.kept_xy = fe->kept_xy.p;
  A.n_kept = fe->n_kept.p, A.hw = fe->hw.p, A.radius = fe->cfg.min_dist, A.f_thresh = (float)fe->cfg.f_threshold;
  A.pnp_pts = fe->pnp_pts.p, A.pnp_ids = fe->pnp_ids.p, A.n_pnp = fe->n_pnp.p;
  A.f_conf = fe->cfg.f_confidence;
  static const bool tu_prof = vio::env_flag("VIO_AMD_TU_PROF");
  if (tu_prof) (void)fe->d_prof.ensure(32);
  A.prof = tu_prof ? fe->d_prof.p : nullptr;
  const bool small = fe->cap <= 256;
  const size_t shm = ((small ? sizeof(TrackShared<256>) : sizeof(TrackShared<kMaxCap>)) + 15 & ~(size_t)15) + sizeof(RansacShared);
  const void *kern = small ? (const void *)track_update_kernel<256> : (const void *)track_update_kernel<kMaxCap>;
  if (!fe->attr_set) {
    HIP_OK(hipFuncSetAttribute(kern, hipFuncAttributeMaxDynamicSharedMemorySize, (int)shm));
    fe->attr_set = true;
  }
  if (A.prof) (void)hipMemsetAsync(A.prof, 0, 32 * sizeof(long long), st);
  if (small) hipLaunchKernelGGL(track_update_kernel<256>, dim3(fe->n_seq), dim3(256), shm, st, A, publish);
  else hipLaunchKernelGGL(track_update_kernel<kMaxCap>, dim3(fe->n_seq), dim3(256), shm, st, A, publish);
  if (A.prof) {
    long long h[32];
    if (hipStreamSynchronize(st) == hipSuccess && hipMemcpy(h, A.prof, sizeof(h), hipMemcpyDeviceToHost) == hipSuccess) {
      static const char *name[11] = {"load", "compact", "ransac(cur,forw)", "compact", "pnp list", "ransac(pre,forw)", "compact", "counts+rank",
                                     "inside bits", "greedy", "outputs"};
      fprintf(stderr, "track_update cycles (sequence 0, publish %d):", publish);
      const int map[11][2] = {{0, 1}, {1, 2}, {2, 3}, {3, 4}, {4, 5}, {5, 6}, {6, 7}, {7, 8}, {8, 9}, {9, 10}, {10, 11}};
      for (int k = 0; k < 11; k++) fprintf(stderr, " %s %lld,", name[k], h[map[k][1]] - h[map[k][0]]);
      fprintf(stderr, " total %lld\n", h[11] - h[0]);
      for (int c = 0; c < 2; c++)
        fprintf(stderr, "   ransac call %d: draw %lld, gather+collinear %lld, 7-point %lld, scoring %lld, scan %lld, mask %lld, rounds %lld\n", c,
                h[16 + 8 * c], h[17 + 8 * c], h[18 + 8 * c], h[19 + 8 * c], h[20 + 8 * c], h[21 + 8 * c], h[22 + 8 * c]);
    }
  }
  return VIO_OK;
}

int fe_step(vio_frontend *fe, const uint8_t *d_frames , int publish, hipStream_t st, bool keep_frames = false) {
  const int S = fe->n_seq, rows = fe->cfg.image_rows, cols = fe->cfg.image_cols, cap = fe->cap;
  const size_t img_bytes = (size_t)rows * cols;
  const int fidx = fe->have_img ? 1 - fe->cur_idx : fe->cur_idx;
  uint8_t *forw = fe->pyr[fidx].p;
  const bool fused0 = fe->ld.levels >= 2 && cols % 4 == 0 && fe->ld.cols[1] % 4 == 0 && cols >= 8 && fe->ld.pyr_bytes % 4 == 0 &&
                      img_bytes % 4 == 0 && (uintptr_t)d_frames % 4 == 0 && (uintptr_t)forw % 4 == 0 && fe->ld.off[1] % 4 == 0;
  const bool alias0 = keep_frames && fused0 && !vio::env_flag("VIO_AMD_COPY_LEVEL0");
  fe->lvl0[fidx] = alias0 ? d_frames : nullptr;
  if (!fused0) {
    const int vec_ok = img_bytes % 16 == 0 && fe->ld.pyr_bytes % 16 == 0 && (uintptr_t)d_frames % 16 == 0 &&
                       (uintptr_t)forw % 16 == 0;
    dim3 grd((unsigned)((img_bytes + 16 * 256 - 1) / (16 * 256)), S);
    hipLaunchKernelGGL(copy_frames_kernel, grd, dim3(256), 0, st, d_frames, img_bytes, forw, fe->ld.pyr_bytes, img_bytes,
                       vec_ok);
  }
  for (int l = 1; l < fe->ld.levels; l++) {
    const uint8_t *sp = forw + fe->ld.off[l - 1];
    uint8_t *dp = forw + fe->ld.off[l];
    const int sc = fe->ld.cols[l - 1], dc = fe->ld.cols[l];
    if (l == 1 && fused0) {
      dim3 blk(256), grd((dc + kPdW - 1) / kPdW, (fe->ld.rows[1] + kPd4H * kPd4T - 1) / (kPd4H * kPd4T), S);
      if (alias0)
        hipLaunchKernelGGL(pyr_down4_kernel<false>, grd, blk, 0, st, d_frames, img_bytes, dp, fe->ld.pyr_bytes, rows, cols, fe->ld.rows[1], dc,
                           (uint8_t *)nullptr);
      else
        hipLaunchKernelGGL(pyr_down4_kernel<true>, grd, blk, 0, st, d_frames, img_bytes, dp, fe->ld.pyr_bytes, rows, cols, fe->ld.rows[1], dc, forw);
      continue;
    }
    const bool dwords = sc % 4 == 0 && dc % 4 == 0 && sc >= 8 && fe->ld.pyr_bytes % 4 == 0 && (uintptr_t)sp % 4 == 0 && (uintptr_t)dp % 4 == 0;
    if (dwords) {
      dim3 blk(256), grd((dc + kPdW - 1) / kPdW, (fe->ld.rows[l] + kPd4H * kPd4T - 1) / (kPd4H * kPd4T), S);
      hipLaunchKernelGGL(pyr_down4_kernel<false>, grd, blk, 0, st, sp, fe->ld.pyr_bytes, dp, fe->ld.pyr_bytes, fe->ld.rows[l - 1], sc, fe->ld.rows[l], dc,
                         (uint8_t *)nullptr);
    } else {
      dim3 blk(256), grd((dc + kPdW - 1) / kPdW, (fe->ld.rows[l] + kPdH - 1) / kPdH, S);
      hipLaunchKernelGGL(pyr_down_kernel, grd, blk, 0, st, sp, dp, fe->ld.pyr_bytes, fe->ld.rows[l - 1], sc, fe->ld.rows[l], dc);
    }
  }
  if (!fe->have_img) {
    fe->have_img = true;
    fe->cur_idx = fidx;
  } else {
    LkParams P;
    P.ld = fe->ld, P.cap = cap;
    P.max_count = std::min(std::max(fe->cfg.lk_max_iters, 0), 100);
    double eps = std::min(std::max(fe->cfg.lk_eps, 0.), 10.);
    P.epsilon_sq = eps * eps, P.epsilon_sq_f = lk_eps_screen(eps * eps), P.min_eig = (float)fe->cfg.lk_min_eig;
    P.prev0 = fe->lvl0[fe->cur_idx], P.next0 = fe->lvl0[fidx], P.stride0 = img_bytes;
    dim3 grd((cap + 3) / 4, S);
    if (fe->lk_stats_on && fe->lk_stats.p)
      hipLaunchKernelGGL((lk_track_kernel<true>), grd, dim3(256), 0, st, fe->pyr[fe->cur_idx].p, forw, P, fe->n_pts.p, fe->cur_pts.p,
                         fe->forw_pts.p, fe->lk_status.p, fe->lk_err.p, fe->lk_stats.p);
    else
      hipLaunchKernelGGL((lk_track_kernel<false>), grd, dim3(256), 0, st, fe->pyr[fe->cur_idx].p, forw, P, fe->n_pts.p, fe->cur_pts.p,
                         fe->forw_pts.p, fe->lk_status.p, fe->lk_err.p, (unsigned long long *)nullptr);
  }
  int rcu = launch_track_update(fe, publish, st);
  if (rcu != VIO_OK) return rcu;
  if (publish) {
    dim3 tb(256), tg((cols + kDetWaves * kDetW - 1) / (kDetWaves * kDetW), fe->nseg, S);
    hipLaunchKernelGGL(detect_kernel<false>, tg, tb, 0, st, alias0 ? d_frames : forw, alias0 ? img_bytes : fe->ld.pyr_bytes, (const uint8_t *)nullptr, (size_t)0,
                       fe->kept_xy.p, fe->n_kept.p, cap, fe->hw.p, fe->cfg.min_dist, fe->max_bits.p, rows, cols, fe->cand.p,
                       fe->seg_cap, fe->n_cand.p, fe->detect_always ? (const int *)nullptr : fe->n_forw.p, fe->cfg.max_corners);
    SelectParams SP;
    SP.cap = cap, SP.rows = rows, SP.cols = cols, SP.max_corners = fe->cfg.max_corners, SP.min_dist = (float)fe->cfg.min_dist;
    SP.fx = fe->cfg.fx, SP.fy = fe->cfg.fy, SP.cx = fe->cfg.cx, SP.cy = fe->cfg.cy;
    hipLaunchKernelGGL(corner_select_kernel, dim3(S), dim3(kSelThreads), 0, st, fe->cand.p, fe->seg_cap, fe->nseg, fe->n_cand.p,
                       fe->max_bits.p, fe->cfg.quality_level, SP, fe->forw_pts.p, fe->cur_pts.p, fe->pre_pts.p, fe->ids.p,
                       fe->track_cnt.p, fe->n_forw.p, fe->n_pts.p, fe->n_id.p, fe->obs.p, fe->n_obs.p);
  }
  HIP_OK(hipGetLastError());
  fe->cur_idx = fidx;
  return VIO_OK;
}

}

extern "C" {

int vio_frontend_create(const VioConfig *cfg, int32_t n_seq, vio_frontend_t **out) {
  if (!cfg || !out || n_seq < 1) return VIO_EINVAL;
  if (cfg->lk_win != kWin || cfg->lk_levels < 0 || cfg->lk_levels >= kMaxLevels || cfg->max_corners < 1 ||
      cfg->max_corners > kMaxCap || cfg->image_rows < 32 || cfg->image_cols < 32 || cfg->min_dist < 0 || cfg->min_dist > kMaxRadius ||
      cfg->image_rows > 32767 || cfg->image_cols > 65535)
    return VIO_EINVAL;
  if (!vio::device_ready("the front-end")) return VIO_ENODEV;
  vio_frontend *fe = new vio_frontend();
  fe->device = vio::current_device();
  fe->cfg = *cfg, fe->n_seq = n_seq, fe->cap = cfg->max_corners;
  fe->detect_always = vio::env_flag("VIO_AMD_DETECT_ALWAYS");
  LevelDims &ld = fe->ld;
  ld.rows[0] = cfg->image_rows, ld.cols[0] = cfg->image_cols, ld.off[0] = 0, ld.levels = 1;
  size_t off = (size_t)ld.rows[0] * ld.cols[0];
  for (int l = 1; l <= cfg->lk_levels; l++) {
    int r = (ld.rows[l - 1] + 1) / 2, c = (ld.cols[l - 1] + 1) / 2;
    if (c <= kWin || r <= kWin) break;
    ld.rows[l] = r, ld.cols[l] = c, ld.off[l] = off, off += (size_t)r * c, ld.levels = l + 1;
  }
  ld.pyr_bytes = (off + 255) & ~(size_t)255;
  const size_t S = n_seq, cap = fe->cap;
  fe->nseg = (cfg->image_rows + kDetR - 1) / kDetR;
  if (fe->nseg > kSelMaxSeg) {
    delete fe;
    return VIO_ECAP;
  }
  fe->seg_cap = kDetR * cfg->image_cols / 4;
  if (hipStreamCreateWithFlags(&fe->stream, hipStreamNonBlocking) != hipSuccess) {
    delete fe;
    return VIO_ENODEV;
  }
  if (fe->pyr[0].ensure(S * ld.pyr_bytes) != VIO_OK || fe->pyr[1].ensure(S * ld.pyr_bytes) != VIO_OK ||
      fe->max_bits.ensure(S * fe->nseg) != VIO_OK || fe->cand.ensure(S * fe->nseg * fe->seg_cap) != VIO_OK ||
      fe->n_cand.ensure(S * fe->nseg) != VIO_OK || fe->cur_pts.ensure(S * cap * 2) != VIO_OK ||
      fe->pre_pts.ensure(S * cap * 2) != VIO_OK || fe->forw_pts.ensure(S * cap * 2) != VIO_OK || fe->lk_err.ensure(S * cap) != VIO_OK ||
      fe->ids.ensure(S * cap) != VIO_OK || fe->track_cnt.ensure(S * cap) != VIO_OK || fe->n_pts.ensure(S) != VIO_OK ||
      fe->n_forw.ensure(S) != VIO_OK || fe->n_id.ensure(S) != VIO_OK || fe->kept_xy.ensure(S * cap * 2) != VIO_OK ||
      fe->n_kept.ensure(S) != VIO_OK || fe->pnp_pts.ensure(S * cap * 2) != VIO_OK || fe->pnp_ids.ensure(S * cap) != VIO_OK ||
      fe->n_pnp.ensure(S) != VIO_OK || fe->n_obs.ensure(S) != VIO_OK || fe->lk_status.ensure(S * cap) != VIO_OK ||
      fe->obs.ensure(S * cap) != VIO_OK || fe->hw.ensure((size_t)2 * cfg->min_dist + 1) != VIO_OK) {
    delete fe;
    return VIO_ENOMEM;
  }
  std::vector<int> hw;
  circle_halfwidths(cfg->min_dist, hw);
  if (hipMemcpy(fe->hw.p, hw.data(), hw.size() * sizeof(int), hipMemcpyHostToDevice) != hipSuccess ||
      hipMemset(fe->max_bits.p, 0, sizeof(unsigned) * S * fe->nseg) != hipSuccess ||
      hipMemset(fe->n_cand.p, 0, sizeof(int) * S * fe->nseg) != hipSuccess || hipMemset(fe->n_pts.p, 0, sizeof(int) * S) != hipSuccess ||
      hipMemset(fe->n_forw.p, 0, sizeof(int) * S) != hipSuccess || hipMemset(fe->n_id.p, 0, sizeof(int) * S) != hipSuccess ||
      hipMemset(fe->n_kept.p, 0, sizeof(int) * S) != hipSuccess || hipMemset(fe->n_pnp.p, 0, sizeof(int) * S) != hipSuccess ||
      hipMemset(fe->n_obs.p, 0, sizeof(int) * S) != hipSuccess) {
    delete fe;
    return VIO_ENODEV;
  }
  *out = fe;
  return VIO_OK;
}

int vio_frontend_get_device(const vio_frontend_t *fe, int32_t *device) {
  if (!fe || !device) return VIO_EINVAL;
  *device = fe->device;
  return VIO_OK;
}

void vio_frontend_destroy(vio_frontend_t *fe) {
  if (!fe) return;
  vio::DeviceScope scope(fe->device);
  delete fe;
}

int vio_frontend_upload_frames(vio_frontend_t *fe, const uint8_t *gray, int32_t n_frames, int32_t rows, int32_t cols,
                               int32_t stride) {
  if (!fe || !gray || n_frames < 1) return VIO_EINVAL;
  if (rows != fe->cfg.image_rows || cols != fe->cfg.image_cols || stride < cols) return VIO_EINVAL;
  VIO_ON_DEVICE_OF(fe);
  const size_t px = (size_t)rows * cols, total = (size_t)n_frames * fe->n_seq;
  if (fe->pending) return VIO_ESTATE;
  HIP_OK(hipDeviceSynchronize());
  for (int k = 0; k < 2; k++) {
    if (fe->lvl0[k])
      HIP_OK(hipMemcpy2D(fe->pyr[k].p, fe->ld.pyr_bytes, fe->lvl0[k], px, px, fe->n_seq, hipMemcpyDeviceToDevice));
    fe->lvl0[k] = nullptr;
  }
  fe->frames.release();
  if (fe->frames.ensure(total * px) != VIO_OK) return VIO_ENOMEM;
  HIP_OK(hipMemcpy2D(fe->frames.p, cols, gray, stride, cols, total * rows, hipMemcpyHostToDevice));
  fe->n_frames = n_frames;
  return VIO_OK;
}

int vio_frontend_step_resident(vio_frontend_t *fe, int32_t frame_index, int32_t publish, void *stream) {
  if (!fe) return VIO_EINVAL;
  if (!fe->frames.p || frame_index < 0 || frame_index >= fe->n_frames) return VIO_ESTATE;
  if (fe->pending) return VIO_ESTATE;
  VIO_ON_DEVICE_OF(fe);
  hipStream_t st = stream ? (hipStream_t)stream : fe->stream;
  int rc = fe->timer.begin(st);
  if (rc != VIO_OK) return rc;
  const size_t px = (size_t)fe->cfg.image_rows * fe->cfg.image_cols;
  rc = fe_step(fe, fe->frames.p + (size_t)frame_index * fe->n_seq * px, publish, st, true);
  if (rc != VIO_OK) return rc;
  return fe->timer.end(st);
}

int vio_frontend_sync(vio_frontend_t *fe) {
  if (!fe) return VIO_EINVAL;
  VIO_ON_DEVICE_OF(fe);
  HIP_OK(hipDeviceSynchronize());
  return VIO_OK;
}

int vio_frontend_kernel_ms(vio_frontend_t *fe, double *ms_avg, int32_t *launches) {
  if (!fe || !ms_avg || !launches) return VIO_EINVAL;
  VIO_ON_DEVICE_OF(fe);
  HIP_OK(hipDeviceSynchronize());
  return fe->timer.drain(ms_avg, launches);
}

namespace {
struct HostRange {
  const uint8_t *p;
  size_t n;
};
std::mutex g_host_reg_m;
std::vector<HostRange> g_host_reg;
bool host_range_registered(const void *ptr, size_t bytes) {
  const uint8_t *b = static_cast<const uint8_t *>(ptr);
  std::lock_guard<std::mutex> lk(g_host_reg_m);
  for (const HostRange &r : g_host_reg)
    if (b >= r.p && b + bytes <= r.p + r.n) return true;
  return false;
}
}

int vio_host_register(void *ptr, size_t bytes) {
  if (!ptr || bytes == 0) return VIO_EINVAL;
  if (!vio::device_ready("host-buffer registration")) return VIO_ENODEV;
  {
    std::lock_guard<std::mutex> lk(g_host_reg_m);
    const uint8_t *b = static_cast<const uint8_t *>(ptr);
    for (const HostRange &r : g_host_reg)
      if (b < r.p + r.n && r.p < b + bytes) return VIO_ESTATE;
  }
  if (hipHostRegister(ptr, bytes, hipHostRegisterPortable) != hipSuccess) {
    (void)hipGetLastError();
    return VIO_ENOMEM;
  }
  std::lock_guard<std::mutex> lk(g_host_reg_m);
  g_host_reg.push_back({static_cast<const uint8_t *>(ptr), bytes});
  return VIO_OK;
}

int vio_host_unregister(void *ptr) {
  if (!ptr) return VIO_EINVAL;
  {
    std::lock_guard<std::mutex> lk(g_host_reg_m);
    size_t i = 0;
    for (; i < g_host_reg.size(); i++)
      if (g_host_reg[i].p == static_cast<const uint8_t *>(ptr)) break;
    if (i == g_host_reg.size()) return VIO_ESTATE;
    g_host_reg.erase(g_host_reg.begin() + (long)i);
  }
  if (hipDeviceSynchronize() != hipSuccess || hipHostUnregister(ptr) != hipSuccess) {
    (void)hipGetLastError();
    return VIO_ENODEV;
  }
  return VIO_OK;
}

static int submit_body(vio_frontend_t *fe, const uint8_t *gray, int32_t rows, int32_t cols, int32_t stride, int32_t publish) {
  VIO_ON_DEVICE_OF(fe);
  const size_t px = (size_t)rows * cols, S = fe->n_seq;
  if (fe->d_stage.ensure(S * px) != VIO_OK) return VIO_ENOMEM;
  if (fe->p_obs.ensure(S * fe->cap) != VIO_OK || fe->p_nobs.ensure(S) != VIO_OK) return VIO_ENOMEM;
  hipStream_t st = fe->stream;
  if (stride == cols && host_range_registered(gray, S * px)) {
    HIP_OK(hipMemcpyAsync(fe->d_stage.p, gray, S * px, hipMemcpyHostToDevice, st));
  } else {
    if (fe->p_frames.ensure(S * px) != VIO_OK) return VIO_ENOMEM;
    const size_t n_chunks = S >= 32 ? 8 : 1, per = (S + n_chunks - 1) / n_chunks;
    for (size_t c0 = 0; c0 < S; c0 += per) {
      const size_t c1 = std::min(S, c0 + per);
      vio::HostPool::get().parallel_for((int)(c1 - c0), [&](int i) {
        const size_t s = c0 + i;
        const uint8_t *src = gray + s * (size_t)rows * stride;
        uint8_t *dst = fe->p_frames.p + s * px;
        if (stride == cols) memcpy(dst, src, px);
        else
          for (int r = 0; r < rows; r++) memcpy(dst + (size_t)r * cols, src + (size_t)r * stride, cols);
      });
      HIP_OK(hipMemcpyAsync(fe->d_stage.p + c0 * px, fe->p_frames.p + c0 * px, (c1 - c0) * px, hipMemcpyHostToDevice, st));
    }
  }
  int rc = fe_step(fe, fe->d_stage.p, publish, st);
  if (rc != VIO_OK) return rc;
  if (publish) {
    HIP_OK(hipMemcpyAsync(fe->p_obs.p, fe->obs.p, sizeof(VioObs) * S * fe->cap, hipMemcpyDeviceToHost, st));
    HIP_OK(hipMemcpyAsync(fe->p_nobs.p, fe->n_obs.p, sizeof(int) * S, hipMemcpyDeviceToHost, st));
  }
  return VIO_OK;
}

int vio_frontend_submit_images(vio_frontend_t *fe, const uint8_t *gray, int32_t rows, int32_t cols, int32_t stride, int32_t publish) {
  if (!fe || !gray) return VIO_EINVAL;
  if (rows != fe->cfg.image_rows || cols != fe->cfg.image_cols || stride < cols) return VIO_EINVAL;
  if (fe->pending) return VIO_ESTATE;
  const int rc = submit_body(fe, gray, rows, cols, stride, publish);
  if (rc != VIO_OK) return rc;
  fe->pending = true, fe->pending_publish = publish != 0, fe->pending_async = false;
  return VIO_OK;
}

int vio_frontend_submit_images_async(vio_frontend_t *fe, const uint8_t *gray, int32_t rows, int32_t cols, int32_t stride, int32_t publish) {
  if (!fe || !gray) return VIO_EINVAL;
  if (rows != fe->cfg.image_rows || cols != fe->cfg.image_cols || stride < cols) return VIO_EINVAL;
  if (fe->pending) return VIO_ESTATE;
  try {
    if (!fe->async) {
      fe->async = new vio_frontend::Async();
      vio_frontend::Async *a = fe->async;
      a->th = std::thread([fe, a] {
        for (;;) {
          std::unique_lock<std::mutex> lk(a->m);
          a->cv.wait(lk, [&] { return a->quit || a->has_job; });
          if (a->quit) return;
          a->has_job = false;
          lk.unlock();
          const int rc = submit_body(fe, a->gray, a->rows, a->cols, a->stride, a->publish);
          lk.lock();
          a->rc = rc, a->busy = false;
          lk.unlock();
          a->cv.notify_all();
        }
      });
    }
  } catch (...) {
    return VIO_ENOMEM;
  }
  vio_frontend::Async *a = fe->async;
  {
    std::lock_guard<std::mutex> lk(a->m);
    a->gray = gray, a->rows = rows, a->cols = cols, a->stride = stride, a->publish = publish;
    a->has_job = true, a->busy = true, a->rc = VIO_OK;
  }
  a->cv.notify_all();
  fe->pending = true, fe->pending_publish = publish != 0, fe->pending_async = true;
  return VIO_OK;
}

int vio_frontend_collect(vio_frontend_t *fe, VioObs *out_obs, int32_t *n_obs) {
  if (!fe || !n_obs) return VIO_EINVAL;
  if (!fe->pending) return VIO_ESTATE;
  if (fe->pending_publish && !out_obs) return VIO_EINVAL;
  if (fe->async && fe->pending_async) {
    vio_frontend::Async *a = fe->async;
    std::unique_lock<std::mutex> lk(a->m);
    a->cv.wait(lk, [&] { return !a->busy; });
    if (a->rc != VIO_OK) {
      fe->pending = false;
      return a->rc;
    }
  }
  VIO_ON_DEVICE_OF(fe);
  fe->pending = false;
  HIP_OK(hipStreamSynchronize(fe->stream));
  const size_t S = fe->n_seq;
  for (size_t s = 0; s < S; s++) n_obs[s] = 0;
  if (fe->pending_publish)
    for (size_t s = 0; s < S; s++) {
      n_obs[s] = fe->p_nobs.p[s];
      memcpy(out_obs + s * fe->cap, fe->p_obs.p + s * fe->cap, sizeof(VioObs) * fe->p_nobs.p[s]);
    }
  return VIO_OK;
}

int vio_frontend_read_images(vio_frontend_t *fe, const uint8_t *gray, int32_t rows, int32_t cols, int32_t stride,
                             const double *headers, int32_t publish, VioObs *out_obs, int32_t *n_obs) {
  (void)headers;
  if (!fe || !gray || !n_obs || (publish && !out_obs)) return VIO_EINVAL;
  int rc = vio_frontend_submit_images(fe, gray, rows, cols, stride, publish);
  if (rc != VIO_OK) return rc;
  return vio_frontend_collect(fe, out_obs, n_obs);
}

int vio_frontend_read_image(vio_frontend_t *fe, int32_t seq, const uint8_t *gray, int32_t rows, int32_t cols, int32_t stride,
                            double header, int32_t publish, VioObs *out_obs, int32_t *n_obs, VioTrackViz *viz) {
  (void)seq, (void)viz;
  if (!fe || fe->n_seq != 1 || seq != 0) return VIO_EINVAL;
  return vio_frontend_read_images(fe, gray, rows, cols, stride, &header, publish, out_obs, n_obs);
}

int vio_frontend_get_state(vio_frontend_t *fe, int32_t seq, float *cur_pts, int32_t *ids, int32_t *track_cnt, int32_t cap,
                           int32_t *n) {
  if (!fe || seq < 0 || seq >= fe->n_seq || !n) return VIO_EINVAL;
  if (fe->pending) return VIO_ESTATE;
  VIO_ON_DEVICE_OF(fe);
  HIP_OK(hipDeviceSynchronize());
  int m = 0;
  HIP_OK(hipMemcpy(&m, fe->n_pts.p + seq, sizeof(int), hipMemcpyDeviceToHost));
  *n = m;
  if (m > cap) return VIO_ECAP;
  const size_t base = (size_t)seq * fe->cap;
  if (m > 0) {
    HIP_OK(hipMemcpy(cur_pts, fe->cur_pts.p + base * 2, sizeof(float) * 2 * m, hipMemcpyDeviceToHost));
    HIP_OK(hipMemcpy(ids, fe->ids.p + base, sizeof(int) * m, hipMemcpyDeviceToHost));
    HIP_OK(hipMemcpy(track_cnt, fe->track_cnt.p + base, sizeof(int) * m, hipMemcpyDeviceToHost));
  }
  return VIO_OK;
}

int vio_frontend_lk_iterations(vio_frontend_t *fe, int32_t enable, uint64_t *iterations, uint64_t *visits, int32_t levels_cap) {
  if (!fe || (iterations && (!visits || levels_cap < 1))) return VIO_EINVAL;
  if (fe->pending) return VIO_ESTATE;
  VIO_ON_DEVICE_OF(fe);
  constexpr int kSlots = 16 * 64;
  if (!fe->lk_stats.p) {
    if (fe->lk_stats.ensure(kSlots) != VIO_OK) return VIO_ENOMEM;
    HIP_OK(hipMemset(fe->lk_stats.p, 0, sizeof(unsigned long long) * kSlots));
  }
  HIP_OK(hipStreamSynchronize(fe->stream));
  if (iterations) {
    unsigned long long h[kSlots];
    HIP_OK(hipMemcpy(h, fe->lk_stats.p, sizeof(h), hipMemcpyDeviceToHost));
    const int L = fe->ld.levels;
    for (int l = 0; l < levels_cap; l++) {
      iterations[l] = visits[l] = 0;
      for (int c = 0; c < 64 && l < L; c++) iterations[l] += h[16 * c + l], visits[l] += h[16 * c + L + l];
    }
    HIP_OK(hipMemset(fe->lk_stats.p, 0, sizeof(h)));
  }
  if (enable >= 0) fe->lk_stats_on = enable != 0;
  return VIO_OK;
}

int vio_frontend_get_pnp_points(vio_frontend_t *fe, int32_t seq, float *forw_pts, int32_t *ids, int32_t cap, int32_t *n) {
  if (!fe || seq < 0 || seq >= fe->n_seq || !n) return VIO_EINVAL;
  if (fe->pending) return VIO_ESTATE;
  VIO_ON_DEVICE_OF(fe);
  HIP_OK(hipDeviceSynchronize());
  int m = 0;
  HIP_OK(hipMemcpy(&m, fe->n_pnp.p + seq, sizeof(int), hipMemcpyDeviceToHost));
  *n = m;
  if (m > cap) return VIO_ECAP;
  const size_t base = (size_t)seq * fe->cap;
  if (m > 0) {
    if (!forw_pts || !ids) return VIO_EINVAL;
    HIP_OK(hipMemcpy(forw_pts, fe->pnp_pts.p + base * 2, sizeof(float) * 2 * m, hipMemcpyDeviceToHost));
    HIP_OK(hipMemcpy(ids, fe->pnp_ids.p + base, sizeof(int) * m, hipMemcpyDeviceToHost));
  }
  return VIO_OK;
}

int vio_frontend_set_tracks(vio_frontend_t *fe, int32_t seq, int32_t n, const float *pre_pts, const float *cur_pts,
                            const float *forw_pts, const int32_t *ids, const int32_t *track_cnt, const uint8_t *lk_status) {
  if (!fe || seq < 0 || seq >= fe->n_seq || n < 0 || (n > 0 && (!pre_pts || !cur_pts || !forw_pts || !ids || !track_cnt || !lk_status)))
    return VIO_EINVAL;
  if (n > fe->cap) return VIO_ECAP;
  if (fe->pending) return VIO_ESTATE;
  VIO_ON_DEVICE_OF(fe);
  HIP_OK(hipDeviceSynchronize());
  const size_t base = (size_t)seq * fe->cap;
  if (n > 0) {
    HIP_OK(hipMemcpy(fe->pre_pts.p + base * 2, pre_pts, sizeof(float) * 2 * n, hipMemcpyHostToDevice));
    HIP_OK(hipMemcpy(fe->cur_pts.p + base * 2, cur_pts, sizeof(float) * 2 * n, hipMemcpyHostToDevice));
    HIP_OK(hipMemcpy(fe->forw_pts.p + base * 2, forw_pts, sizeof(float) * 2 * n, hipMemcpyHostToDevice));
    HIP_OK(hipMemcpy(fe->ids.p + base, ids, sizeof(int) * n, hipMemcpyHostToDevice));
    HIP_OK(hipMemcpy(fe->track_cnt.p + base, track_cnt, sizeof(int) * n, hipMemcpyHostToDevice));
    HIP_OK(hipMemcpy(fe->lk_status.p + base, lk_status, n, hipMemcpyHostToDevice));
  }
  HIP_OK(hipMemcpy(fe->n_pts.p + seq, &n, sizeof(int), hipMemcpyHostToDevice));
  return VIO_OK;
}

int vio_frontend_update_tracks(vio_frontend_t *fe, int32_t publish) {
  if (!fe) return VIO_EINVAL;
  if (fe->pending) return VIO_ESTATE;
  VIO_ON_DEVICE_OF(fe);
  int rc = launch_track_update(fe, publish, fe->stream);
  if (rc != VIO_OK) return rc;
  HIP_OK(hipStreamSynchronize(fe->stream));
  HIP_OK(hipGetLastError());
  return VIO_OK;
}

int vio_frontend_get_tracks(vio_frontend_t *fe, int32_t seq, float *forw_pts, int32_t *ids, int32_t *track_cnt, int32_t cap,
                            int32_t *n) {
  if (!fe || seq < 0 || seq >= fe->n_seq || !n) return VIO_EINVAL;
  if (fe->pending) return VIO_ESTATE;
  VIO_ON_DEVICE_OF(fe);
  HIP_OK(hipDeviceSynchronize());
  int m = 0;
  HIP_OK(hipMemcpy(&m, fe->n_forw.p + seq, sizeof(int), hipMemcpyDeviceToHost));
  *n = m;
  if (m > cap) return VIO_ECAP;
  const size_t base = (size_t)seq * fe->cap;
  if (m > 0) {
    HIP_OK(hipMemcpy(forw_pts, fe->forw_pts.p + base * 2, sizeof(float) * 2 * m, hipMemcpyDeviceToHost));
    HIP_OK(hipMemcpy(ids, fe->ids.p + base, sizeof(int) * m, hipMemcpyDeviceToHost));
    HIP_OK(hipMemcpy(track_cnt, fe->track_cnt.p + base, sizeof(int) * m, hipMemcpyDeviceToHost));
  }
  return VIO_OK;
}

using FrontendPtr = std::unique_ptr<vio_frontend, void (*)(vio_frontend_t *)>;

int vio_klt_track(const VioConfig *cfg, const uint8_t *prev, const uint8_t *next, int32_t rows, int32_t cols, int32_t stride,
                  const float *prev_pts, int32_t n, float *next_pts, uint8_t *status, float *err) {
  if (!cfg || !prev || !next || n < 0 || (n > 0 && (!prev_pts || !next_pts || !status || !err))) return VIO_EINVAL;
  if (n == 0) return VIO_OK;
  VioConfig c = *cfg;
  c.image_rows = rows, c.image_cols = cols, c.max_corners = std::min(std::max(n, 1), kMaxCap);
  if (n > kMaxCap) return VIO_ECAP;
  vio_frontend *raw = nullptr;
  int rc = vio_frontend_create(&c, 1, &raw);
  if (rc != VIO_OK) return rc;
  const FrontendPtr fe(raw, vio_frontend_destroy);
  const size_t px = (size_t)rows * cols;
  DevBuf<uint8_t> d;
  if (d.ensure(2 * px) != VIO_OK) return VIO_ENOMEM;
  if (hipMemcpy2D(d.p, cols, prev, stride, cols, rows, hipMemcpyHostToDevice) != hipSuccess) return VIO_ENODEV;
  if (hipMemcpy2D(d.p + px, cols, next, stride, cols, rows, hipMemcpyHostToDevice) != hipSuccess) return VIO_ENODEV;
  hipStream_t st = fe->stream;
  for (int k = 0; k < 2; k++) {
    uint8_t *dst = fe->pyr[k].p;
    if (hipMemcpyAsync(dst, d.p + k * px, px, hipMemcpyDeviceToDevice, st) != hipSuccess) return VIO_ENODEV;
    for (int l = 1; l < fe->ld.levels; l++) {
      dim3 blk(256), grd((fe->ld.cols[l] + kPdW - 1) / kPdW, (fe->ld.rows[l] + kPdH - 1) / kPdH, 1);
      hipLaunchKernelGGL(pyr_down_kernel, grd, blk, 0, st, dst + fe->ld.off[l - 1], dst + fe->ld.off[l], fe->ld.pyr_bytes,
                         fe->ld.rows[l - 1], fe->ld.cols[l - 1], fe->ld.rows[l], fe->ld.cols[l]);
    }
  }
  if (hipMemcpyAsync(fe->cur_pts.p, prev_pts, sizeof(float) * 2 * n, hipMemcpyHostToDevice, st) != hipSuccess) return VIO_ENODEV;
  if (hipMemcpyAsync(fe->n_pts.p, &n, sizeof(int), hipMemcpyHostToDevice, st) != hipSuccess) return VIO_ENODEV;
  LkParams P;
  P.ld = fe->ld, P.cap = fe->cap, P.max_count = std::min(std::max(c.lk_max_iters, 0), 100);
  double eps = std::min(std::max(c.lk_eps, 0.), 10.);
  P.epsilon_sq = eps * eps, P.epsilon_sq_f = lk_eps_screen(eps * eps), P.min_eig = (float)c.lk_min_eig;
  P.prev0 = P.next0 = nullptr, P.stride0 = 0;
  hipLaunchKernelGGL((lk_track_kernel<false>), dim3((fe->cap + 3) / 4, 1), dim3(256), 0, st, fe->pyr[0].p, fe->pyr[1].p, P, fe->n_pts.p,
                     fe->cur_pts.p, fe->forw_pts.p, fe->lk_status.p, fe->lk_err.p, (unsigned long long *)nullptr);
  if (hipStreamSynchronize(st) != hipSuccess || hipGetLastError() != hipSuccess) return VIO_ENODEV;
  if (hipMemcpy(next_pts, fe->forw_pts.p, sizeof(float) * 2 * n, hipMemcpyDeviceToHost) != hipSuccess) return VIO_ENODEV;
  if (hipMemcpy(status, fe->lk_status.p, n, hipMemcpyDeviceToHost) != hipSuccess) return VIO_ENODEV;
  if (hipMemcpy(err, fe->lk_err.p, sizeof(float) * n, hipMemcpyDeviceToHost) != hipSuccess) return VIO_ENODEV;
  return VIO_OK;
}

int vio_good_features(const VioConfig *cfg, const uint8_t *img, const uint8_t *mask, int32_t rows, int32_t cols, int32_t stride,
                      int32_t max_corners, float *corners, int32_t *n_corners) {
  if (!cfg || !img || !corners || !n_corners || max_corners < 1) return VIO_EINVAL;
  if (max_corners > kMaxCap) return VIO_ECAP;
  VioConfig c = *cfg;
  c.image_rows = rows, c.image_cols = cols, c.max_corners = max_corners;
  vio_frontend *raw = nullptr;
  int rc = vio_frontend_create(&c, 1, &raw);
  if (rc != VIO_OK) return rc;
  const FrontendPtr fe(raw, vio_frontend_destroy);
  const size_t px = (size_t)rows * cols;
  hipStream_t st = fe->stream;
  if (hipMemcpy2D(fe->pyr[0].p, cols, img, stride, cols, rows, hipMemcpyHostToDevice) != hipSuccess) return VIO_ENODEV;
  if (fe->mask.ensure(px) != VIO_OK) return VIO_ENOMEM;
  if (mask) {
    if (hipMemcpy2D(fe->mask.p, cols, mask, stride, cols, rows, hipMemcpyHostToDevice) != hipSuccess) return VIO_ENODEV;
  } else if (hipMemset(fe->mask.p, 255, px) != hipSuccess) {
    return VIO_ENODEV;
  }
  if (hipMemset(fe->max_bits.p, 0, sizeof(unsigned) * fe->nseg) != hipSuccess ||
      hipMemset(fe->n_cand.p, 0, sizeof(int) * fe->nseg) != hipSuccess)
    return VIO_ENODEV;
  dim3 tb(256), tg((cols + kDetWaves * kDetW - 1) / (kDetWaves * kDetW), fe->nseg, 1);
  hipLaunchKernelGGL(detect_kernel<true>, tg, tb, 0, st, fe->pyr[0].p, fe->ld.pyr_bytes, fe->mask.p, px, fe->kept_xy.p, fe->n_kept.p,
                     fe->cap, fe->hw.p, c.min_dist, fe->max_bits.p, rows, cols, fe->cand.p, fe->seg_cap, fe->n_cand.p, (const int *)nullptr, 0);
  SelectParams SP;
  SP.cap = fe->cap, SP.rows = rows, SP.cols = cols, SP.max_corners = max_corners, SP.min_dist = (float)c.min_dist;
  SP.fx = c.fx, SP.fy = c.fy, SP.cx = c.cx, SP.cy = c.cy;
  hipLaunchKernelGGL(corner_select_kernel, dim3(1), dim3(kSelThreads), 0, st, fe->cand.p, fe->seg_cap, fe->nseg, fe->n_cand.p, fe->max_bits.p,
                     c.quality_level, SP, fe->forw_pts.p, fe->cur_pts.p, fe->pre_pts.p, fe->ids.p, fe->track_cnt.p, fe->n_forw.p, fe->n_pts.p,
                     fe->n_id.p, fe->obs.p, fe->n_obs.p);
  if (hipStreamSynchronize(st) != hipSuccess || hipGetLastError() != hipSuccess) return VIO_ENODEV;
  int n = 0;
  if (hipMemcpy(&n, fe->n_pts.p, sizeof(int), hipMemcpyDeviceToHost) != hipSuccess) return VIO_ENODEV;
  *n_corners = n;
  if (n > 0 && hipMemcpy(corners, fe->forw_pts.p, sizeof(float) * 2 * n, hipMemcpyDeviceToHost) != hipSuccess) return VIO_ENODEV;
  return VIO_OK;
}

__global__ __launch_bounds__(256) void ransac_only_kernel(const float *p1, const float *p2, int n, float thresh, double conf,
                                                          uint8_t *mask) {
  extern __shared__ __attribute__((aligned(16))) unsigned char smem_raw[];
  RansacShared &R = *reinterpret_cast<RansacShared *>(smem_raw);
  fundamental_ransac_block(R, p1, p2, n, thresh, conf, mask);
}

int vio_fundamental_ransac(const VioConfig *cfg, const float *pts1, const float *pts2, int32_t n, uint8_t *inlier_mask) {
  if (!cfg || !pts1 || !pts2 || !inlier_mask || n < 0) return VIO_EINVAL;
  if (n == 0) return VIO_OK;
  int ndev = 0;
  if (hipGetDeviceCount(&ndev) != hipSuccess || ndev < 1) return VIO_ENODEV;
  DevBuf<float> d1, d2;
  DevBuf<uint8_t> dm;
  if (d1.ensure((size_t)2 * n) != VIO_OK || d2.ensure((size_t)2 * n) != VIO_OK || dm.ensure((size_t)n) != VIO_OK) return VIO_ENOMEM;
  if (hipMemcpy(d1.p, pts1, sizeof(float) * 2 * n, hipMemcpyHostToDevice) != hipSuccess) return VIO_ENODEV;
  if (hipMemcpy(d2.p, pts2, sizeof(float) * 2 * n, hipMemcpyHostToDevice) != hipSuccess) return VIO_ENODEV;
  hipLaunchKernelGGL(ransac_only_kernel, dim3(1), dim3(256), sizeof(RansacShared), 0, d1.p, d2.p, n, (float)cfg->f_threshold,
                     cfg->f_confidence, dm.p);
  if (hipDeviceSynchronize() != hipSuccess || hipGetLastError() != hipSuccess) return VIO_ENODEV;
  if (hipMemcpy(inlier_mask, dm.p, n, hipMemcpyDeviceToHost) != hipSuccess) return VIO_ENODEV;
  return VIO_OK;
}

}

__global__ __launch_bounds__(256) void ransac_batch_kernel(const float *p1, const float *p2, const int *count, int stride, int min_count,
                                                           float thresh, double conf, uint8_t *mask) {
  extern __shared__ __attribute__((aligned(16))) unsigned char smem_raw[];
  RansacShared &R = *reinterpret_cast<RansacShared *>(smem_raw);
  const int p = blockIdx.x, n = count[p];
  if (n < min_count || n > stride) return;
  fundamental_ransac_block(R, p1 + 2 * (size_t)p * stride, p2 + 2 * (size_t)p * stride, n, thresh, conf, mask + (size_t)p * stride);
}

namespace vio {
int fundamental_ransac_batch(hipStream_t st, const float *p1, const float *p2, const int *count, int n_prob, int stride, int min_count,
                             float thresh, double conf, uint8_t *mask) {
  if (n_prob < 1) return VIO_OK;
  hipLaunchKernelGGL(ransac_batch_kernel, dim3(n_prob), dim3(256), sizeof(RansacShared), st, p1, p2, count, stride, min_count, thresh, conf,
                     mask);
  HIP_OK(hipGetLastError());
  return VIO_OK;
}
}
```

Baseline: 181,900.

## Index-compact tracker lists, pack RANSAC points, parallelize corner selection outputs

The tracker compaction now builds an index list instead of copying every per-point array twice, and RANSAC reads points through a packed float4 accessor. Corner selection uses wave ballots in place of per-element atomics, and assigns new ids and writes outputs in parallel instead of through a single thread. The change also adds correctly-rounded double-double acos/cos/pow for the cubic solver in the LMedS path, plus optional cycle profiling. It cuts shared-memory traffic and serial loops, but the exact-math path adds cost whenever it runs.

Result: faster. 185,600, median of 6 (+2.0%).

```diff
diff --git a/vins-mobile_amd/csrc/vio_exact_math.h b/vins-mobile_amd/csrc/vio_exact_math.h
--- /dev/null
+++ b/vins-mobile_amd/csrc/vio_exact_math.h
@@ -0,0 +1,94 @@
+#pragma once
+#include <math.h>
+#if defined(__HIPCC__) || defined(__CUDACC__)
+#define VIO_XM_HD __host__ __device__ inline
+#define VIO_XM_CONST static constexpr
+#else
+#define VIO_XM_HD inline
+#define VIO_XM_CONST static constexpr
+#endif
+namespace vio_xm {
+struct dd { double h, l; };
+VIO_XM_HD dd two_sum(double a, double b) { double s = a + b, bb = s - a; return {s, (a - (s - bb)) + (b - bb)}; }
+VIO_XM_HD dd fast_two_sum(double a, double b) { double s = a + b; return {s, b - (s - a)}; }
+VIO_XM_HD dd two_prod(double a, double b) { double p = a * b; return {p, fma(a, b, -p)}; }
+VIO_XM_HD dd add(dd a, dd b) {
+  dd s = two_sum(a.h, b.h), t = two_sum(a.l, b.l);
+  s = fast_two_sum(s.h, s.l + t.h);
+  return fast_two_sum(s.h, s.l + t.l);
+}
+VIO_XM_HD dd add_d(dd a, double b) { dd s = two_sum(a.h, b); return fast_two_sum(s.h, s.l + a.l); }
+VIO_XM_HD dd mul(dd a, dd b) { dd p = two_prod(a.h, b.h); return fast_two_sum(p.h, p.l + (a.h * b.l + a.l * b.h)); }
+VIO_XM_HD dd mul_d(dd a, double b) { dd p = two_prod(a.h, b); return fast_two_sum(p.h, p.l + a.l * b); }
+VIO_XM_HD dd neg(dd a) { return {-a.h, -a.l}; }
+VIO_XM_CONST double kPio2[3] = {0x1.921fb54442d18p+0, 0x1.1a62633145c07p-54, -0x1.f1976b7ed8fbcp-110};
+VIO_XM_CONST double kLn2[3] = {0x1.62e42fefa39efp-1, 0x1.abc9e3b39803fp-56, 0x1.7b57a079a1934p-111};
+VIO_XM_CONST double kSinC[14][2] = {{0x1.0000000000000p+0, 0x0.0p+0}, {-0x1.5555555555555p-3, -0x1.5555555555555p-57}, {0x1.1111111111111p-7, 0x1.1111111111111p-63}, {-0x1.a01a01a01a01ap-13, -0x1.a01a01a01a01ap-73}, {0x1.71de3a556c734p-19, -0x1.c154f8ddc6c00p-73}, {-0x1.ae64567f544e4p-26, 0x1.c062e06d1f209p-80}, {0x1.6124613a86d09p-33, 0x1.f28e0cc748ebep-87}, {-0x1.ae7f3e733b81fp-41, -0x1.1d8656b0ee8cbp-97}, {0x1.952c77030ad4ap-49, 0x1.ac981465ddc6cp-103}, {-0x1.2f49b46814157p-57, -0x1.2650f61dbdcb4p-112}, {0x1.71b8ef6dcf572p-66, -0x1.d043ae40c4647p-120}, {-0x1.761b41316381ap-75, 0x1.3423c7d91404fp-130}, {0x1.3f3ccdd165fa9p-84, -0x1.58ddadf344487p-139}, {-0x1.d1ab1c2dccea3p-94, -0x1.054d0c78aea14p-149}};
+VIO_XM_CONST double kCosC[14][2] = {{0x1.0000000000000p+0, 0x0.0p+0}, {-0x1.0000000000000p-1, 0x0.0p+0}, {0x1.5555555555555p-5, 0x1.5555555555555p-59}, {-0x1.6c16c16c16c17p-10, 0x1.f49f49f49f49fp-65}, {0x1.a01a01a01a01ap-16, 0x1.a01a01a01a01ap-76}, {-0x1.27e4fb7789f5cp-22, -0x1.cbbc05b4fa99ap-76}, {0x1.1eed8eff8d898p-29, -0x1.2aec959e14c06p-83}, {-0x1.93974a8c07c9dp-37, -0x1.05d6f8a2efd1fp-92}, {0x1.ae7f3e733b81fp-45, 0x1.1d8656b0ee8cbp-101}, {-0x1.6827863b97d97p-53, -0x1.eec01221a8b0bp-107}, {0x1.e542ba4020225p-62, 0x1.ea72b4afe3c2fp-120}, {-0x1.0ce396db7f853p-70, 0x1.aebcdbd20331cp-124}, {0x1.f2cf01972f578p-80, -0x1.9ada5fcc1ab14p-135}, {-0x1.88e85fc6a4e5ap-89, 0x1.71c37ebd16540p-143}};
+VIO_XM_CONST double kExpC[12][2] = {{0x1.0000000000000p+0, 0x0.0p+0}, {0x1.0000000000000p+0, 0x0.0p+0}, {0x1.0000000000000p-1, 0x0.0p+0}, {0x1.5555555555555p-3, 0x1.5555555555555p-57}, {0x1.5555555555555p-5, 0x1.5555555555555p-59}, {0x1.1111111111111p-7, 0x1.1111111111111p-63}, {0x1.6c16c16c16c17p-10, -0x1.f49f49f49f49fp-65}, {0x1.a01a01a01a01ap-13, 0x1.a01a01a01a01ap-73}, {0x1.a01a01a01a01ap-16, 0x1.a01a01a01a01ap-76}, {0x1.71de3a556c734p-19, -0x1.c154f8ddc6c00p-73}, {0x1.27e4fb7789f5cp-22, 0x1.cbbc05b4fa99ap-76}, {0x1.ae64567f544e4p-26, -0x1.c062e06d1f209p-80}};
+VIO_XM_HD dd reduce(dd x, double k, const double c[3]) {
+  dd r = add(x, neg(two_prod(k, c[0])));
+  r = add(r, neg(two_prod(k, c[1])));
+  return add_d(r, -(k * c[2]));
+}
+VIO_XM_HD void sincos_kernel(dd r, dd &s, dd &c) {
+  const dd r2 = mul(r, r);
+  double ts = kSinC[13][0], tc = kCosC[13][0];
+  for (int n = 12; n >= 6; n--) ts = ts * r2.h + kSinC[n][0], tc = tc * r2.h + kCosC[n][0];
+  dd as = {ts, 0.0}, ac = {tc, 0.0};
+  for (int n = 5; n >= 0; n--) {
+    as = add(mul(as, r2), dd{kSinC[n][0], kSinC[n][1]});
+    ac = add(mul(ac, r2), dd{kCosC[n][0], kCosC[n][1]});
+  }
+  s = mul(as, r), c = ac;
+}
+VIO_XM_HD dd cos_dd(double x) {
+  const double k = nearbyint(x * 0.63661977236758138);
+  dd s, c;
+  sincos_kernel(reduce(dd{x, 0.0}, k, kPio2), s, c);
+  const int q = (int)k & 3;
+  return q == 0 ? c : q == 1 ? neg(s) : q == 2 ? neg(c) : s;
+}
+VIO_XM_HD dd sin_dd(double x) {
+  const double k = nearbyint(x * 0.63661977236758138);
+  dd s, c;
+  sincos_kernel(reduce(dd{x, 0.0}, k, kPio2), s, c);
+  const int q = (int)k & 3;
+  return q == 0 ? s : q == 1 ? c : q == 2 ? neg(s) : neg(c);
+}
+VIO_XM_HD double cos_cr(double x) {
+  if (!(fabs(x) < 1048576.0)) return cos(x);
+  return cos_dd(x).h;
+}
+VIO_XM_HD double acos_cr(double v) {
+  if (!(fabs(v) < 1.0)) return acos(v);
+  const double a0 = acos(v);
+  const dd f = add_d(cos_dd(a0), -v);
+  const double sn = sin_dd(a0).h;
+  const dd corr = {f.h / sn, 0.0};
+  const dd rem = add(f, neg(mul_d(dd{sn, 0.0}, corr.h)));
+  return add_d(dd{corr.h, rem.h / sn}, a0).h;
+}
+VIO_XM_HD dd exp_dd(dd p, int &e2) {
+  const double k = nearbyint(p.h * 1.4426950408889634);
+  dd r = reduce(p, k, kLn2);
+  r.h *= 0.03125, r.l *= 0.03125;
+  double t = kExpC[11][0];
+  for (int n = 10; n >= 5; n--) t = t * r.h + kExpC[n][0];
+  dd a = {t, 0.0};
+  for (int n = 4; n >= 0; n--) a = add(mul(a, r), dd{kExpC[n][0], kExpC[n][1]});
+  for (int q = 0; q < 5; q++) a = mul(a, a);
+  e2 = (int)k;
+  return a;
+}
+VIO_XM_HD double pow_cr(double x, double y) {
+  const double l0 = log(x);
+  if (!(x > 0.0) || !(fabs(l0) < 600.0) || !(fabs(y) < 1.0)) return pow(x, y);
+  int e2;
+  const dd em = exp_dd(dd{-l0, 0.0}, e2);
+  const dd z = add_d(mul_d(em, ldexp(x, e2)), -1.0);
+  const dd L = add_d(add_d(z, -0.5 * z.h * z.h), l0);
+  const dd r = exp_dd(mul_d(L, y), e2);
+  return ldexp(r.h, e2);
+}
+}
diff --git a/vins-mobile_amd/csrc/vio_frontend.hip b/vins-mobile_amd/csrc/vio_frontend.hip
--- a/vins-mobile_amd/csrc/vio_frontend.hip
+++ b/vins-mobile_amd/csrc/vio_frontend.hip
@@ -1,6 +1,8 @@
 #include <hip/hip_runtime.h>
 
 #include <type_traits>
+
+#include "vio_exact_math.h"
 
 #include <math.h>
 #include <stdint.h>
@@ -504,7 +506,10 @@
   }
 }
 
-__device__ int solve_cubic_dev(const double c[4], double r[3]) {
+__device__ __attribute__((noinline)) double exact_fn(int which, double x) {
+  return which == 0 ? vio_xm::acos_cr(x) : which == 1 ? vio_xm::cos_cr(x) : vio_xm::pow_cr(x, 0.333333333333);
+}
+__device__ int solve_cubic_dev(const double c[4], double r[3], bool exact) {
   double a0 = c[0], a1 = c[1], a2 = c[2], a3 = c[3];
   double x0 = 0, x1 = 0, x2 = 0;
   int n = 0;
@@ -528,13 +533,16 @@
     double Qcubed = Q * Q * Q, d = Qcubed - R * R;
     const double kPi = 3.14159265358979323846;
     if (d >= 0) {
-      double theta = acos(R / sqrt(Qcubed)), sqrtQ = sqrt(Q);
+      const double av = R / sqrt(Qcubed);
+      double theta = exact ? exact_fn(0, av) : acos(av), sqrtQ = sqrt(Q);
       double t0 = -2 * sqrtQ, t1 = theta * (1. / 3), t2 = a1 * (1. / 3);
-      x0 = t0 * cos(t1) - t2, x1 = t0 * cos(t1 + (2. * kPi / 3)) - t2, x2 = t0 * cos(t1 + (4. * kPi / 3)) - t2;
+      const double g0 = t1, g1 = t1 + (2. * kPi / 3), g2 = t1 + (4. * kPi / 3);
+      if (exact) x0 = t0 * exact_fn(1, g0) - t2, x1 = t0 * exact_fn(1, g1) - t2, x2 = t0 * exact_fn(1, g2) - t2;
+      else x0 = t0 * cos(g0) - t2, x1 = t0 * cos(g1) - t2, x2 = t0 * cos(g2) - t2;
       n = 3;
     } else {
       d = sqrt(-d);
-      double e = pow(d + fabs(R), 0.333333333333);
+      double e = exact ? exact_fn(2, d + fabs(R)) : pow(d + fabs(R), 0.333333333333);
       if (R > 0) e = -e;
       x0 = (e + Q / e) - a1 * (1. / 3);
       n = 1;
@@ -549,7 +557,7 @@
   int colperm[10];
 };
 
-__device__ __forceinline__ int run7point_group(const float *ms1, const float *ms2, double *fmatrix, SevenPointWork &wk, int l) {
+__device__ __forceinline__ int run7point_group(const float *ms1, const float *ms2, double *fmatrix, SevenPointWork &wk, int l, bool exact) {
   double *a = wk.a, *f1 = wk.f1, *f2 = wk.f2;
   int *colperm = wk.colperm;
   auto group_sync = [] {
@@ -645,7 +653,7 @@
            f2[6] * (f1[1] * f1[5] - f1[2] * f1[4]) - f2[7] * (f1[0] * f1[5] - f1[2] * f1[3]) +
            f2[8] * (f1[0] * f1[4] - f1[1] * f1[3]);
     c[0] = f1[0] * t0 - f1[1] * t1 + f1[2] * t2;
-    n = solve_cubic_dev(c, r);
+    n = solve_cubic_dev(c, r, exact);
     if (n >= 1 && n <= 3)
       for (int k = 0; k < n; k++, fmatrix += 9) {
         double lambda = r[k], mu = 1., s = f1[8] * r[k] + f2[8];
@@ -709,9 +717,13 @@
   double med[kHypBatch][3], min_median;
 };
 
-template <class MaskT>
-__device__ void fundamental_ransac_block(RansacShared &S, const float *m1, const float *m2, int count, float thresh,
-                                         double confidence, MaskT *mask, long long *prof = nullptr) {
+struct GlobalPts {
+  const float *m1, *m2;
+  __device__ __forceinline__ float4 operator()(int i) const { return make_float4(m1[2 * i], m1[2 * i + 1], m2[2 * i], m2[2 * i + 1]); }
+};
+template <class MaskT, class Pts>
+__device__ __forceinline__ void fundamental_ransac_block(RansacShared &S, const Pts pts, int count, float thresh, double confidence,
+                                                         MaskT *mask, long long *prof = nullptr) {
   const int tid = threadIdx.x, nt = blockDim.x;
   long long pt = prof ? clock64() : 0;
 #define RS_STAMP(k)                                                    \
@@ -752,8 +764,9 @@
               if (idx_i == idx[j]) break;
             if (j == i) break;
           }
-          S.ms1[h][2 * i] = m1[2 * idx_i], S.ms1[h][2 * i + 1] = m1[2 * idx_i + 1];
-          S.ms2[h][2 * i] = m2[2 * idx_i], S.ms2[h][2 * i + 1] = m2[2 * idx_i + 1];
+          const float4 q = pts(idx_i);
+          S.ms1[h][2 * i] = q.x, S.ms1[h][2 * i + 1] = q.y;
+          S.ms2[h][2 * i] = q.z, S.ms2[h][2 * i + 1] = q.w;
           i++;
         }
         if (with_check && i == model_points && (have_collinear_dev(S.ms1[h], i) || have_collinear_dev(S.ms2[h], i))) continue;
@@ -789,9 +802,10 @@
     __syncthreads();
     RS_STAMP(0);
     for (int it = tid; it < nb * 7; it += nt) {
-      const int h = it / 7, i = it - 7 * h, id = S.idx[h][i];
-      S.ms1[h][2 * i] = m1[2 * id], S.ms1[h][2 * i + 1] = m1[2 * id + 1];
-      S.ms2[h][2 * i] = m2[2 * id], S.ms2[h][2 * i + 1] = m2[2 * id + 1];
+      const int h = it / 7, i = it - 7 * h;
+      const float4 q = pts(S.idx[h][i]);
+      S.ms1[h][2 * i] = q.x, S.ms1[h][2 * i + 1] = q.y;
+      S.ms2[h][2 * i] = q.z, S.ms2[h][2 * i + 1] = q.w;
     }
     __syncthreads();
     if (tid < nb) S.coll[tid] = (have_collinear_dev(S.ms1[tid], 7) || have_collinear_dev(S.ms2[tid], 7)) ? 1 : 0;
@@ -816,7 +830,7 @@
     RS_STAMP(1);
     for (int h = tid >> 4; h < nb; h += nt >> 4) {
       int n = 0;
-      if (S.valid[h]) n = run7point_group(S.ms1[h], S.ms2[h], S.F[h], S.work[h], tid & 15);
+      if (S.valid[h]) n = run7point_group(S.ms1[h], S.ms2[h], S.F[h], S.work[h], tid & 15, lmeds);
       if ((tid & 15) == 0) {
         S.nmodels[h] = n < 0 ? 0 : n;
         S.good[h][0] = S.good[h][1] = S.good[h][2] = 0;
@@ -830,7 +844,8 @@
         if (k >= S.nmodels[h]) continue;
         int bits[14];
         for (int i = 0; i < count; i++) {
-          const int b = __float_as_int(epipolar_error(S.F[h] + 9 * k, m1[2 * i], m1[2 * i + 1], m2[2 * i], m2[2 * i + 1]));
+          const float4 q = pts(i);
+          const int b = __float_as_int(epipolar_error(S.F[h] + 9 * k, q.x, q.y, q.z, q.w));
           int j = i;
           for (; j > 0 && bits[j - 1] > b; j--) bits[j] = bits[j - 1];
           bits[j] = b;
@@ -842,8 +857,10 @@
     for (int item = tid; item < nb * 3 * count; item += nt) {
       int hk = item / count, i = item - hk * count;
       int h = hk / 3, k = hk - 3 * h;
-      if (k < S.nmodels[h] && epipolar_inlier(S.F[h] + 9 * k, m1[2 * i], m1[2 * i + 1], m2[2 * i], m2[2 * i + 1], t))
-        atomicAdd(&S.good[h][k], 1);
+      if (k < S.nmodels[h]) {
+        const float4 q = pts(i);
+        if (epipolar_inlier(S.F[h] + 9 * k, q.x, q.y, q.z, q.w, t)) atomicAdd(&S.good[h][k], 1);
+      }
     }
     __syncthreads();
     RS_STAMP(3);
@@ -884,11 +901,15 @@
     double sigma = 2.5 * 1.4826 * (1 + 5. / (count - model_points)) * sqrt(S.min_median);
     sigma = fmax(sigma, 0.001);
     const float ts = (float)(sigma * sigma);
-    for (int i = tid; i < count; i += nt)
-      mask[i] = epipolar_inlier(S.bestF, m1[2 * i], m1[2 * i + 1], m2[2 * i], m2[2 * i + 1], ts) ? 1 : 0;
+    for (int i = tid; i < count; i += nt) {
+      const float4 q = pts(i);
+      mask[i] = epipolar_inlier(S.bestF, q.x, q.y, q.z, q.w, ts) ? 1 : 0;
+    }
   } else if (!lmeds && S.max_good > 0 && !S.failed_first) {
-    for (int i = tid; i < count; i += nt)
-      mask[i] = epipolar_inlier(S.bestF, m1[2 * i], m1[2 * i + 1], m2[2 * i], m2[2 * i + 1], t) ? 1 : 0;
+    for (int i = tid; i < count; i += nt) {
+      const float4 q = pts(i);
+      mask[i] = epipolar_inlier(S.bestF, q.x, q.y, q.z, q.w, t) ? 1 : 0;
+    }
   } else {
     for (int i = tid; i < count; i += nt) mask[i] = 1;
   }
@@ -922,61 +943,49 @@
   float pre[CAP][2], cur[CAP][2], forw[CAP][2];
   int ids[CAP], cnt[CAP];
   int keep[CAP];
+  int idx[CAP];
   int pos[CAP];
-  float t_pre[CAP][2], t_cur[CAP][2], t_forw[CAP][2];
-  int t_ids[CAP], t_cnt[CAP];
+  float4 pack[CAP];
   int n;
   int order[CAP];
+  int ncnt[CAP];
   int ixy[CAP][2];
   unsigned long long inside[CAP][CAP / 64];
   int hw[2 * kMaxRadius + 1];
 };
 
-template <int CAP>
-__device__ void compact_block(TrackShared<CAP> &T) {
+template <int CAP, bool FIRST>
+__device__ __forceinline__ void shorten_list(TrackShared<CAP> &T) {
+  __shared__ int s_wcnt[16];
   const int tid = threadIdx.x, nt = blockDim.x;
+  const int wave = tid >> 6, lane = tid & 63, nwv = nt >> 6;
   const int n = T.n;
+  int running = 0;
+  for (int base = 0; base < n; base += nt) {
+    const int i = base + tid;
+    const bool k = i < n && T.keep[i];
+    const int v = FIRST ? i : (i < n ? T.idx[i] : 0);
+    const unsigned long long b = __builtin_amdgcn_ballot_w64(k);
+    if (lane == 0) s_wcnt[wave] = __builtin_popcountll(b);
+    __syncthreads();
+    int off = running, total = 0;
+    for (int w = 0; w < nwv; w++) {
+      const int c = s_wcnt[w];
+      if (w < wave) off += c;
+      total += c;
+    }
+    if (k) T.idx[off + __builtin_popcountll(b & ((1ull << lane) - 1ull))] = v;
+    running += total;
+    if (base + nt < n) __syncthreads();
+  }
+  if (tid == 0) T.n = running;
   __syncthreads();
-  {
-    __shared__ int s_wcnt[16];
-    const int wave = tid >> 6, lane = tid & 63, nwv = nt >> 6;
-    int running = 0;
-    for (int base = 0; base < n; base += nt) {
-      const int i = base + tid;
-      const bool k = i < n && T.keep[i];
-      const unsigned long long b = __builtin_amdgcn_ballot_w64(k);
-      if (lane == 0) s_wcnt[wave] = __builtin_popcountll(b);
-      __syncthreads();
-      int off = running, total = 0;
-      for (int w = 0; w < nwv; w++) {
-        const int c = s_wcnt[w];
-        if (w < wave) off += c;
-        total += c;
-      }
-      if (i < n) T.pos[i] = off + __builtin_popcountll(b & ((1ull << lane) - 1ull));
-      running += total;
-      __syncthreads();
-    }
-    if (tid == 0) T.n = running;
-  }
-  __syncthreads();
-  for (int i = tid; i < n; i += nt)
-    if (T.keep[i]) {
-      int p = T.pos[i];
-      T.t_pre[p][0] = T.pre[i][0], T.t_pre[p][1] = T.pre[i][1];
-      T.t_cur[p][0] = T.cur[i][0], T.t_cur[p][1] = T.cur[i][1];
-      T.t_forw[p][0] = T.forw[i][0], T.t_forw[p][1] = T.forw[i][1];
-      T.t_ids[p] = T.ids[i], T.t_cnt[p] = T.cnt[i];
-    }
-  __syncthreads();
-  for (int i = tid; i < T.n; i += nt) {
-    T.pre[i][0] = T.t_pre[i][0], T.pre[i][1] = T.t_pre[i][1];
-    T.cur[i][0] = T.t_cur[i][0], T.cur[i][1] = T.t_cur[i][1];
-    T.forw[i][0] = T.t_forw[i][0], T.forw[i][1] = T.t_forw[i][1];
-    T.ids[i] = T.t_ids[i], T.cnt[i] = T.t_cnt[i];
-  }
-  __syncthreads();
-}
+}
+
+struct PackedPts {
+  const float4 *pack;
+  __device__ __forceinline__ float4 operator()(int i) const { return pack[i]; }
+};
 
 template <int CAP>
 __global__ __launch_bounds__(256, 2) void track_update_kernel(TrackerArrays A, int publish) {
@@ -1003,38 +1012,46 @@
   }
   __syncthreads();
   TU_STAMP(1);
-  if (n0 > 0) {
-    compact_block(T);
-    TU_STAMP(2);
-    if (T.n >= 8) {
-      fundamental_ransac_block(R, &T.cur[0][0], &T.forw[0][0], T.n, A.f_thresh, A.f_conf, T.keep, A.prof && seq == 0 ? A.prof + 16 : nullptr);
-      TU_STAMP(3);
-      compact_block(T);
-    }
-  }
-  TU_STAMP(4);
-  for (int i = tid; i < T.n; i += nt) {
-    A.pnp_pts[(base + i) * 2] = T.forw[i][0], A.pnp_pts[(base + i) * 2 + 1] = T.forw[i][1];
-    A.pnp_ids[base + i] = T.ids[i];
-  }
-  if (tid == 0) A.n_pnp[seq] = T.n;
+  shorten_list<CAP, true>(T);
+  TU_STAMP(2);
+  const int npass = publish ? 2 : 1;
+#pragma nounroll
+  for (int pass = 0; pass < npass; pass++) {
+    if (pass) TU_STAMP(5);
+    const int np = T.n;
+    if (np >= 8) {
+      const float(*from)[2] = pass ? T.pre : T.cur;
+      for (int i = tid; i < np; i += nt) {
+        const int o = T.idx[i];
+        T.pack[i] = make_float4(from[o][0], from[o][1], T.forw[o][0], T.forw[o][1]);
+      }
+      __syncthreads();
+      fundamental_ransac_block(R, PackedPts{T.pack}, np, A.f_thresh, A.f_conf, T.keep, A.prof && seq == 0 ? A.prof + 16 + 8 * pass : nullptr);
+      TU_STAMP(pass ? 6 : 3);
+      shorten_list<CAP, false>(T);
+    }
+    if (pass == 0) {
+      TU_STAMP(4);
+      for (int i = tid; i < T.n; i += nt) {
+        const int o = T.idx[i];
+        A.pnp_pts[(base + i) * 2] = T.forw[o][0], A.pnp_pts[(base + i) * 2 + 1] = T.forw[o][1];
+        A.pnp_ids[base + i] = T.ids[o];
+      }
+      if (tid == 0) A.n_pnp[seq] = T.n;
+    }
+  }
+  const int n = T.n;
   if (publish) {
-    if (T.n >= 8) {
-      TU_STAMP(5);
-      fundamental_ransac_block(R, &T.pre[0][0], &T.forw[0][0], T.n, A.f_thresh, A.f_conf, T.keep, A.prof && seq == 0 ? A.prof + 24 : nullptr);
-      TU_STAMP(6);
-      compact_block(T);
-    }
     TU_STAMP(7);
-    const int n = T.n;
     for (int i = tid; i < n; i += nt) {
-      T.cnt[i] += 1;
-      T.ixy[i][0] = __float2int_rn(T.forw[i][0]), T.ixy[i][1] = __float2int_rn(T.forw[i][1]);
+      const int o = T.idx[i];
+      T.ncnt[i] = T.cnt[o] + 1;
+      T.ixy[i][0] = __float2int_rn(T.forw[o][0]), T.ixy[i][1] = __float2int_rn(T.forw[o][1]);
     }
     __syncthreads();
     for (int i = tid; i < n; i += nt) {
-      int rank = 0, ci = T.cnt[i];
-      for (int j = 0; j < n; j++) rank += (T.cnt[j] > ci || (T.cnt[j] == ci && j < i)) ? 1 : 0;
+      int rank = 0, ci = T.ncnt[i];
+      for (int j = 0; j < n; j++) rank += (T.ncnt[j] > ci || (T.ncnt[j] == ci && j < i)) ? 1 : 0;
       T.order[rank] = i;
     }
     const int words = (n + 63) / 64;
@@ -1106,31 +1123,21 @@
     TU_STAMP(10);
     for (int i = tid; i < n; i += nt)
       if (T.keep[i]) {
-        int p = T.pos[i];
-        T.t_forw[p][0] = T.forw[i][0], T.t_forw[p][1] = T.forw[i][1];
-        T.t_ids[p] = T.ids[i], T.t_cnt[p] = T.cnt[i];
+        const int p = T.pos[i], o = T.idx[i];
+        A.forw_pts[(base + p) * 2] = T.forw[o][0], A.forw_pts[(base + p) * 2 + 1] = T.forw[o][1];
+        A.ids[base + p] = T.ids[o], A.track_cnt[base + p] = T.ncnt[i];
         A.kept_xy[(base + p) * 2] = T.ixy[i][0], A.kept_xy[(base + p) * 2 + 1] = T.ixy[i][1];
       }
-    __syncthreads();
-    for (int i = tid; i < T.n; i += nt) {
-      T.forw[i][0] = T.t_forw[i][0], T.forw[i][1] = T.t_forw[i][1];
-      T.ids[i] = T.t_ids[i], T.cnt[i] = T.t_cnt[i];
-    }
-    if (tid == 0) A.n_kept[seq] = T.n;
-    __syncthreads();
-  }
-  const int n = T.n;
-  for (int i = tid; i < n; i += nt) {
-    A.forw_pts[(base + i) * 2] = T.forw[i][0], A.forw_pts[(base + i) * 2 + 1] = T.forw[i][1];
-    A.ids[base + i] = T.ids[i], A.track_cnt[base + i] = T.cnt[i];
-    if (!publish) {
-      A.pre_pts[(base + i) * 2] = T.pre[i][0], A.pre_pts[(base + i) * 2 + 1] = T.pre[i][1];
-      A.cur_pts[(base + i) * 2] = T.forw[i][0], A.cur_pts[(base + i) * 2 + 1] = T.forw[i][1];
-    }
-  }
-  if (tid == 0) {
-    A.n_forw[seq] = n;
-    if (!publish) A.n_pts[seq] = n;
+    if (tid == 0) A.n_kept[seq] = T.n, A.n_forw[seq] = T.n;
+  } else {
+    for (int i = tid; i < n; i += nt) {
+      const int o = T.idx[i];
+      A.forw_pts[(base + i) * 2] = T.forw[o][0], A.forw_pts[(base + i) * 2 + 1] = T.forw[o][1];
+      A.ids[base + i] = T.ids[o], A.track_cnt[base + i] = T.cnt[o];
+      A.pre_pts[(base + i) * 2] = T.pre[o][0], A.pre_pts[(base + i) * 2 + 1] = T.pre[o][1];
+      A.cur_pts[(base + i) * 2] = T.forw[o][0], A.cur_pts[(base + i) * 2 + 1] = T.forw[o][1];
+    }
+    if (tid == 0) A.n_forw[seq] = n, A.n_pts[seq] = n;
   }
   TU_STAMP(11);
 #undef TU_STAMP
@@ -1347,39 +1354,76 @@
                                                                     double quality, SelectParams P, float *forw_pts,
                                                                     float *cur_pts, float *pre_pts, int *ids, int *track_cnt,
                                                                     int *n_forw, int *n_pts, int *n_id, VioObs *obs,
-                                                                    int *n_obs) {
+                                                                    int *n_obs, long long *prof) {
+#define CS_STAMP(k)                                                  \
+  do {                                                               \
+    if (prof && blockIdx.x == 0 && threadIdx.x == 0) prof[k] = clock64(); \
+  } while (0)
+  CS_STAMP(0);
   __shared__ unsigned long long keys[kSelLds];
-  __shared__ unsigned long long red[kSelThreads / 64];
+  __shared__ unsigned long long red[2][kSelThreads / 64];
   __shared__ int s_n, s_cnt;
+  __shared__ unsigned s_mb;
   __shared__ int s_off[kSelMaxSeg + 1];
+  __shared__ unsigned s_pick[kMaxCap];
+  __shared__ int s_wnew[kSelThreads / 64];
+  static_assert(kMaxCap <= kSelThreads, "the id pass gives every feature slot its own work-item");
   const int seq = blockIdx.x, tid = threadIdx.x, nt = blockDim.x;
+  const int lane = tid & 63, wave = tid >> 6;
   unsigned long long *cand = cand_base + (size_t)seq * nseg * seg_cap;
   const size_t base = (size_t)seq * P.cap;
-  int n = n_forw[seq];
+  const int n_old = n_forw[seq];
+  int n = n_old;
   const int want = P.max_corners - n;
   const float md2 = P.min_dist * P.min_dist;
-  unsigned mb = 0;
-  for (int g = 0; g < nseg; g++) mb = max(mb, max_bits[(size_t)seq * nseg + g]);
+  const int nid0 = n_id[seq];
+  int my_id = -1;
+  float my_x = 0.f, my_y = 0.f;
+  if (tid < n_old) my_id = ids[base + tid], my_x = forw_pts[(base + tid) * 2], my_y = forw_pts[(base + tid) * 2 + 1];
+  if (wave == 0) {
+    int carry = 0;
+    unsigned mb = 0;
+    for (int g0 = 0; g0 < nseg; g0 += 64) {
+      const int g = g0 + lane;
+      const int c = g < nseg ? min(n_cand[(size_t)seq * nseg + g], seg_cap) : 0;
+      mb = max(mb, g < nseg ? max_bits[(size_t)seq * nseg + g] : 0u);
+      int incl = c;
+#pragma unroll
+      for (int o = 1; o < 64; o <<= 1) {
+        const int t = __shfl_up(incl, o, 64);
+        incl += lane >= o ? t : 0;
+      }
+      if (g < nseg) s_off[g] = carry + incl - c;
+      carry += __shfl(incl, 63, 64);
+    }
+#pragma unroll
+    for (int o = 32; o > 0; o >>= 1) mb = max(mb, (unsigned)__shfl_xor((int)mb, o, 64));
+    if (lane == 0) s_off[nseg] = carry, s_mb = mb, s_n = n, s_cnt = 0;
+  }
+  __syncthreads();
+  const unsigned mb = s_mb;
   const float thr = mb ? (float)((double)from_ordered_bits(mb) * quality) : 3.4e38f;
-  if (tid == 0) s_n = n, s_cnt = 0;
+  const int real = s_off[nseg];
+  int sg = 0;
+  for (int i0 = 0; i0 < real; i0 += nt) {
+    const int i = i0 + tid;
+    unsigned long long k = 0;
+    if (i < real) {
+      while (s_off[sg + 1] <= i) sg++;
+      k = cand[(size_t)sg * seg_cap + (i - s_off[sg])];
+    }
+    const bool ok = k && __uint_as_float((unsigned)(k >> 32)) > thr;
+    const unsigned long long b = __builtin_amdgcn_ballot_w64(ok);
+    if (b) {
+      int slot0 = 0;
+      if (lane == 0) slot0 = atomicAdd(&s_cnt, __builtin_popcountll(b));
+      slot0 = __builtin_amdgcn_readfirstlane(slot0);
+      const int slot = slot0 + __builtin_popcountll(b & ((1ull << lane) - 1ull));
+      if (ok && slot < kSelLds) keys[slot] = k;
+    }
+  }
   __syncthreads();
-  if (tid == 0) {
-    int o = 0;
-    for (int g = 0; g < nseg; g++) s_off[g] = o, o += min(n_cand[(size_t)seq * nseg + g], seg_cap);
-    s_off[nseg] = o;
-  }
-  __syncthreads();
-  const int real = s_off[nseg];
-  for (int i = tid; i < real; i += nt) {
-    int g = 0;
-    while (s_off[g + 1] <= i) g++;
-    const unsigned long long k = cand[(size_t)g * seg_cap + (i - s_off[g])];
-    if (k && __uint_as_float((unsigned)(k >> 32)) > thr) {
-      int slot = atomicAdd(&s_cnt, 1);
-      if (slot < kSelLds) keys[slot] = k;
-    }
-  }
-  __syncthreads();
+  CS_STAMP(1);
   for (int g = tid; g < nseg; g += nt) n_cand[(size_t)seq * nseg + g] = 0, max_bits[(size_t)seq * nseg + g] = 0;
   if (s_cnt > kSelLds) {
     __shared__ unsigned long long smax[kSelMaxSeg];
@@ -1432,11 +1476,7 @@
       if (best == 0) break;
       const unsigned bidx = 0xffffffffu - (unsigned)(best & 0xffffffffu);
       const int bx = bidx & 0xffffu, by = bidx >> 16;
-      if (tid == 0) {
-        int p = s_n++;
-        forw_pts[(base + p) * 2] = (float)bx, forw_pts[(base + p) * 2 + 1] = (float)by;
-        ids[base + p] = -1, track_cnt[base + p] = 1;
-      }
+      if (tid == 0) s_pick[s_n++] = bidx;
       const int glo = max(0, (by - reach) / kDetR), ghi = min(nseg - 1, (by + reach) / kDetR);
       for (int g0 = glo; g0 <= ghi; g0 += 4) rescan(g0, min(4, ghi - g0 + 1), bx, by, false);
     }
@@ -1450,19 +1490,16 @@
   }
   for (int round = 0; round < want; round++) {
     unsigned long long best = wave_max_u64(mine);
-    if ((tid & 63) == 0) red[tid >> 6] = best;
+    unsigned long long *rd = red[round & 1];
+    if (lane == 0) rd[wave] = best;
     __syncthreads();
-    best = red[0];
-    for (int w = 1; w < nt / 64; w++) best = red[w] > best ? red[w] : best;
-    __syncthreads();
+    best = rd[0];
+#pragma unroll
+    for (int w = 1; w < kSelThreads / 64; w++) best = rd[w] > best ? rd[w] : best;
     if (best == 0) break;
     const unsigned bidx = 0xffffffffu - (unsigned)(best & 0xffffffffu);
     const int bx = bidx & 0xffffu, by = bidx >> 16;
-    if (tid == 0) {
-      int p = s_n++;
-      forw_pts[(base + p) * 2] = (float)bx, forw_pts[(base + p) * 2 + 1] = (float)by;
-      ids[base + p] = -1, track_cnt[base + p] = 1;
-    }
+    if (tid == 0) s_pick[s_n++] = bidx;
     mine = 0;
     if (P.min_dist >= 1.f) {
       for (int i = tid; i < nc; i += nt) {
@@ -1484,24 +1521,41 @@
   }
   }
   __syncthreads();
+  CS_STAMP(2);
   n = s_n;
-  if (tid == 0) {
-    int nid = n_id[seq];
-    for (int i = 0; i < n; i++)
-      if (ids[base + i] == -1) ids[base + i] = nid++;
-    n_id[seq] = nid;
-    n_forw[seq] = n, n_pts[seq] = n, n_obs[seq] = n;
-  }
+  const bool is_new = tid >= n_old && tid < n;
+  if (is_new) {
+    const unsigned bidx = s_pick[tid];
+    my_x = (float)(int)(bidx & 0xffffu), my_y = (float)(int)(bidx >> 16);
+  }
+  const bool no_id = tid < n && my_id == -1;
+  const unsigned long long nb = __builtin_amdgcn_ballot_w64(no_id);
+  if (lane == 0) s_wnew[wave] = __builtin_popcountll(nb);
   __syncthreads();
-  for (int i = tid; i < n; i += nt) {
-    float x = forw_pts[(base + i) * 2], y = forw_pts[(base + i) * 2 + 1];
+  int before = 0, total = 0;
+#pragma unroll
+  for (int w = 0; w < kSelThreads / 64; w++) {
+    const int c = s_wnew[w];
+    before += w < wave ? c : 0;
+    total += c;
+  }
+  if (no_id) my_id = nid0 + before + __builtin_popcountll(nb & ((1ull << lane) - 1ull));
+  if (tid == 0) n_id[seq] = nid0 + total, n_forw[seq] = n, n_pts[seq] = n, n_obs[seq] = n;
+  CS_STAMP(3);
+  if (tid < n) {
+    const int i = tid;
+    const float x = my_x, y = my_y;
+    if (is_new) forw_pts[(base + i) * 2] = x, forw_pts[(base + i) * 2 + 1] = y, track_cnt[base + i] = 1;
+    if (no_id) ids[base + i] = my_id;
     cur_pts[(base + i) * 2] = x, cur_pts[(base + i) * 2 + 1] = y;
     pre_pts[(base + i) * 2] = x, pre_pts[(base + i) * 2 + 1] = y;
     VioObs o;
-    o.id = ids[base + i];
+    o.id = my_id;
     o.x = ((double)x - P.cx) / P.fx, o.y = ((double)y - P.cy) / P.fy, o.z = 1.0;
     obs[base + i] = o;
   }
+  CS_STAMP(4);
+#undef CS_STAMP
 }
 
 void circle_halfwidths(int radius, std::vector<int> &hw) {
@@ -1548,6 +1602,8 @@
   DevBuf<uint8_t> lk_status;
   DevBuf<VioObs> obs;
   DevBuf<long long> d_prof;
+  DevBuf<long long> d_cs_prof;
+  bool cs_prof = false;
   bool attr_set = false;
   bool detect_always = false;
   DevBuf<uint8_t> frames;
@@ -1803,7 +1859,13 @@
     SP.fx = fe->cfg.fx, SP.fy = fe->cfg.fy, SP.cx = fe->cfg.cx, SP.cy = fe->cfg.cy;
     hipLaunchKernelGGL(corner_select_kernel, dim3(S), dim3(kSelThreads), 0, st, fe->cand.p, fe->seg_cap, fe->nseg, fe->n_cand.p,
                        fe->max_bits.p, fe->cfg.quality_level, SP, fe->forw_pts.p, fe->cur_pts.p, fe->pre_pts.p, fe->ids.p,
-                       fe->track_cnt.p, fe->n_forw.p, fe->n_pts.p, fe->n_id.p, fe->obs.p, fe->n_obs.p);
+                       fe->track_cnt.p, fe->n_forw.p, fe->n_pts.p, fe->n_id.p, fe->obs.p, fe->n_obs.p, fe->cs_prof ? fe->d_cs_prof.p : nullptr);
+    if (fe->cs_prof) {
+      long long h[5];
+      if (hipStreamSynchronize(st) == hipSuccess && hipMemcpy(h, fe->d_cs_prof.p, sizeof(h), hipMemcpyDeviceToHost) == hipSuccess)
+        fprintf(stderr, "corner_select cycles (sequence 0): threshold %lld, selection %lld, ids %lld, outputs %lld, total %lld\n", h[1] - h[0],
+                h[2] - h[1], h[3] - h[2], h[4] - h[3], h[4] - h[0]);
+    }
   }
   HIP_OK(hipGetLastError());
   fe->cur_idx = fidx;
@@ -1825,6 +1887,7 @@
   fe->device = vio::current_device();
   fe->cfg = *cfg, fe->n_seq = n_seq, fe->cap = cfg->max_corners;
   fe->detect_always = vio::env_flag("VIO_AMD_DETECT_ALWAYS");
+  fe->cs_prof = vio::env_flag("VIO_AMD_CS_PROF") && fe->d_cs_prof.ensure(8) == VIO_OK;
   LevelDims &ld = fe->ld;
   ld.rows[0] = cfg->image_rows, ld.cols[0] = cfg->image_cols, ld.off[0] = 0, ld.levels = 1;
   size_t off = (size_t)ld.rows[0] * ld.cols[0];
@@ -2291,7 +2354,7 @@
   SP.fx = c.fx, SP.fy = c.fy, SP.cx = c.cx, SP.cy = c.cy;
   hipLaunchKernelGGL(corner_select_kernel, dim3(1), dim3(kSelThreads), 0, st, fe->cand.p, fe->seg_cap, fe->nseg, fe->n_cand.p, fe->max_bits.p,
                      c.quality_level, SP, fe->forw_pts.p, fe->cur_pts.p, fe->pre_pts.p, fe->ids.p, fe->track_cnt.p, fe->n_forw.p, fe->n_pts.p,
-                     fe->n_id.p, fe->obs.p, fe->n_obs.p);
+                     fe->n_id.p, fe->obs.p, fe->n_obs.p, (long long *)nullptr);
   if (hipStreamSynchronize(st) != hipSuccess || hipGetLastError() != hipSuccess) return VIO_ENODEV;
   int n = 0;
   if (hipMemcpy(&n, fe->n_pts.p, sizeof(int), hipMemcpyDeviceToHost) != hipSuccess) return VIO_ENODEV;
@@ -2304,7 +2367,7 @@
                                                           uint8_t *mask) {
   extern __shared__ __attribute__((aligned(16))) unsigned char smem_raw[];
   RansacShared &R = *reinterpret_cast<RansacShared *>(smem_raw);
-  fundamental_ransac_block(R, p1, p2, n, thresh, conf, mask);
+  fundamental_ransac_block(R, GlobalPts{p1, p2}, n, thresh, conf, mask);
 }
 
 int vio_fundamental_ransac(const VioConfig *cfg, const float *pts1, const float *pts2, int32_t n, uint8_t *inlier_mask) {
@@ -2332,7 +2395,7 @@
   RansacShared &R = *reinterpret_cast<RansacShared *>(smem_raw);
   const int p = blockIdx.x, n = count[p];
   if (n < min_count || n > stride) return;
-  fundamental_ransac_block(R, p1 + 2 * (size_t)p * stride, p2 + 2 * (size_t)p * stride, n, thresh, conf, mask + (size_t)p * stride);
+  fundamental_ransac_block(R, GlobalPts{p1 + 2 * (size_t)p * stride, p2 + 2 * (size_t)p * stride}, n, thresh, conf, mask + (size_t)p * stride);
 }
 
 namespace vio {
```
